# daviyan5/ninpol

Measured on AMD Instinct MI355X. Metric: Mnodes/s interpolated (GLS, 10M-cell hex mesh) + achieved HBM GB/s vs peak, higher is better.
Workload: dtype f64

## Files before the change

include/ninpol_amd.h:

```cpp
#ifndef NINPOL_AMD_H
#define NINPOL_AMD_H

#include <stdint.h>

#ifdef __cplusplus
extern "C" {
#endif

typedef struct nin_grid nin_grid;

enum {
    NIN_OK = 0,
    NIN_EINVAL = -1,
    NIN_ENOMEM = -2,
    NIN_EHIP = -3,
    NIN_ENODEVICE = -4,
    NIN_ERANGE = -5,
    NIN_ESTATE = -6
};

enum { NIN_METHOD_GLS = 0, NIN_METHOD_IDW = 1, NIN_METHOD_LS = 2 };

enum { NIN_I64 = 0, NIN_F64 = 1 };

const char *nin_last_error(void);
const char *nin_version(void);

int nin_grid_create(int64_t dim, int64_t n_elems, int64_t n_points,
                    const int64_t *npoel, const int64_t *nfael, const int64_t *lnofa,
                    const int64_t *lpofa, const int64_t *nedel, const int64_t *lpoed,
                    const int64_t *connectivity, const int64_t *element_types,
                    const double *coords, int coords_dim, int build_edges, int num_threads,
                    nin_grid **out);
void nin_grid_destroy(nin_grid *g);

int nin_grid_create_on_device(int64_t dim, int64_t n_elems, int64_t n_points,
                              const int64_t *npoel, const int64_t *nfael, const int64_t *lnofa,
                              const int64_t *lpofa, const int64_t *nedel, const int64_t *lpoed,
                              const int64_t *connectivity, const int64_t *element_types,
                              const double *coords, int coords_dim, int build_edges, int device,
                              nin_grid **out);

int64_t nin_grid_scalar(const nin_grid *g, const char *name);

int nin_grid_array_info(nin_grid *g, const char *name, int64_t *count, int *dtype);
int nin_grid_array_copy(nin_grid *g, const char *name, void *dst, int64_t count);

int nin_device_count(int *count);
int nin_grid_to_device(nin_grid *g, int device);
int nin_grid_device(const nin_grid *g);

int nin_grid_update_points(nin_grid *g, const double *xyz, int coords_dim);
int nin_grid_update_points_device(nin_grid *g, const double *dev_xyz, int coords_dim, void *stream);
int64_t nin_grid_geometry_updates(const nin_grid *g);
int nin_grid_has_transpose_index(const nin_grid *g);

int nin_fields_set(nin_grid *g, const double *permeability, const double *diff_mag,
                   const double *neumann_flag, const double *neumann_val);

int nin_fields_set_permeability_device(nin_grid *g, const double *dev_permeability, const double *dev_scale, void *stream);
int nin_fields_get_permeability(nin_grid *g, double *permeability, double *diff_mag);
int64_t nin_grid_field_updates(const nin_grid *g);

int nin_fields_scatter_permeability_device(nin_grid *g, const void *dev_cell_ids, int ids_are_int64, int64_t n,
                                           const double *dev_permeability, const double *dev_scale, void *stream);
int nin_weights_dirty_device(nin_grid *g, int method, int add_neumann, double *dev_csr_data, double *dev_neumann_ws, void *stream,
                             int clear, int64_t *n_recomputed);
int64_t nin_grid_dirty_nodes(nin_grid *g);
int nin_grid_dirty_reset(nin_grid *g, int all_dirty, void *stream);

int nin_grid_scatter_points_device(nin_grid *g, const void *dev_node_ids, int ids_are_int64, int64_t n, const double *dev_xyz,
                                   int coords_dim, void *stream);
int nin_grid_scatter_points(nin_grid *g, const int64_t *node_ids, int64_t n, const double *xyz, int coords_dim);

int nin_fields_set_flags_device(nin_grid *g, const void *dev_flags, int flags_are_bytes, void *stream);
int nin_fields_scatter_flags_device(nin_grid *g, const void *dev_node_ids, int ids_are_int64, int64_t n,
                                    const void *dev_flags, int flags_are_bytes, void *stream);
int nin_fields_get_flags(nin_grid *g, uint8_t *neumann );
int64_t nin_grid_flag_updates(const nin_grid *g);

int nin_weights_device(nin_grid *g, int method, const int64_t *targets, int64_t n_targets,
                       int add_neumann, double *dev_csr_data, double *dev_neumann_ws, void *stream);

int nin_weights_host(nin_grid *g, int method, const int64_t *targets, int64_t n_targets,
                     int add_neumann, double *csr_data, double *neumann_ws);

int nin_csr_compact_host(nin_grid *g, const double *dev_csr_data, int32_t *indptr, int32_t *indices,
                         double *data, int64_t *nnz_out, void *stream);

int nin_interpolate_csr_host(nin_grid *g, int method, int32_t *indptr, int32_t *indices, double *data,
                             int64_t *nnz_out, double *neumann_ws);

typedef struct nin_hostmatrix nin_hostmatrix;
int nin_hostmatrix_create(nin_grid *g, int method, nin_hostmatrix **out);
int nin_hostmatrix_full(nin_hostmatrix *m, int32_t *indptr, int32_t *indices, double *data, double *neumann_ws, int64_t *nnz_out,
                        void *stream);
int nin_hostmatrix_update(nin_hostmatrix *m, int clear, void *stream, int64_t *n_rows, int64_t *n_changed, int64_t *n_entries);
int nin_hostmatrix_patch(nin_hostmatrix *m, const int32_t *indptr, int32_t *indices, double *data, double *neumann_ws,
                         int32_t *out_indptr, int32_t *out_indices, double *out_data);
void nin_hostmatrix_destroy(nin_hostmatrix *m);

int nin_csr_patch_rows(int64_t P, const int32_t *indptr, int32_t *indices, double *data, double *neumann_ws, int64_t m,
                       const int32_t *nodes, const int32_t *counts, const int32_t *off, const int32_t *pack_indices,
                       const double *pack_data, const double *pack_nws, int32_t *out_indptr, int32_t *out_indices, double *out_data);

int nin_apply_host(nin_grid *g, int method, const double *u_cells, double *node_values, double *neumann_ws);

int nin_apply_device(nin_grid *g, int method, const double *dev_u_cells, int32_t n_fields, double *dev_node_values,
                     double *dev_neumann_ws, void *stream);
int nin_apply_fields_host(nin_grid *g, int method, const double *u_cells, int32_t n_fields, double *node_values,
                          double *neumann_ws);

int nin_spmv_device(nin_grid *g, const double *dev_csr_data, const double *dev_u_cells, int32_t n_fields, double *dev_node_values,
                    void *stream);
int nin_spmv_transpose_device(nin_grid *g, const double *dev_csr_data, const double *dev_node_values, int32_t n_fields,
                              double *dev_cell_values, void *stream);
int nin_apply_transpose_fields_host(nin_grid *g, int method, const double *node_values, int32_t n_fields, double *cell_values);

int nin_gls_weights_backward_device(nin_grid *g, int add_neumann, const double *dev_grad_csr, const double *dev_grad_neumann_ws,
                                    double *dev_grad_perm, double *dev_grad_diff_mag, void *stream);
int nin_sddmm_device(nin_grid *g, const double *dev_u_cells, const double *dev_node_values, int32_t n_fields, double *dev_grad_csr,
                     void *stream);
int nin_gls_permeability_gradient_host(nin_grid *g, const double *node_values, const double *cell_values, int32_t n_fields,
                                       double *grad_permeability);
int nin_gls_adjoint_plan(nin_grid *g, int64_t counts[4]);
int nin_gls_weights_tangent_device(nin_grid *g, int add_neumann, int32_t n_tangents, const double *dev_tangent_perm,
                                   const double *dev_tangent_diff_mag, double *dev_tangent_csr, double *dev_tangent_neumann_ws,
                                   void *stream);
int nin_gls_permeability_tangent_host(nin_grid *g, const double *tangent_permeability, const double *cell_values, int32_t n_fields,
                                      double *node_values, double *neumann_ws);

int nin_gls_weights_backward_points_device(nin_grid *g, int add_neumann, const double *dev_grad_csr, const double *dev_grad_neumann_ws,
                                           double *dev_grad_points, void *stream);
int nin_gls_points_gradient_host(nin_grid *g, const double *node_values, const double *cell_values, int32_t n_fields,
                                 double *grad_points);

int nin_gls_weights_tangent_points_device(nin_grid *g, int add_neumann, int32_t n_tangents, const double *dev_tangent_points,
                                          double *dev_tangent_csr, double *dev_tangent_neumann_ws, void *stream);
int nin_gls_points_tangent_host(nin_grid *g, const double *tangent_points, const double *cell_values, int32_t n_fields,
                                double *node_values, double *neumann_ws);

typedef struct nin_gls_jacobian nin_gls_jacobian;
int nin_gls_jacobian_create(nin_grid *g, nin_gls_jacobian **out);
int nin_gls_jacobian_linearize(nin_gls_jacobian *J, const double *dev_u_cells, const double *dev_neumann_values, void *stream);
int nin_gls_jacobian_apply(nin_gls_jacobian *J, int32_t n, const double *dev_dperm, const double *dev_ddiff_mag, double *dev_dnode,
                           void *stream);
int nin_gls_jacobian_apply_transpose(nin_gls_jacobian *J, int32_t n, const double *dev_v, double *dev_grad_perm,
                                     double *dev_grad_diff_mag, void *stream);
int nin_gls_jacobian_contrib(nin_gls_jacobian *J, const double **dev_contrib, const double **dev_fold);
int nin_gls_jacobian_stamp(const nin_gls_jacobian *J, int64_t stamp[3]);
void nin_gls_jacobian_destroy(nin_gls_jacobian *J);
int nin_gls_jacobian_linearize_host(nin_gls_jacobian *J, const double *u_cells, const double *neumann_values);
int nin_gls_jacobian_apply_host(nin_gls_jacobian *J, int32_t n, const double *dperm, const double *ddiff_mag, double *dnode);
int nin_gls_jacobian_apply_transpose_host(nin_gls_jacobian *J, int32_t n, const double *v, double *grad_perm, double *grad_diff_mag);
int nin_gls_jacobian_fetch_host(nin_gls_jacobian *J, double *contrib, double *fold);

typedef struct nin_gls_rjacobian nin_gls_rjacobian;
int nin_gls_rjacobian_create(nin_grid *g, int32_t n_params, nin_gls_rjacobian **out);
int nin_gls_rjacobian_linearize(nin_gls_rjacobian *J, const double *dev_u_cells, const double *dev_neumann_values, const double *dev_basis,
                                int32_t basis_per_cell, void *stream);
int nin_gls_rjacobian_apply(nin_gls_rjacobian *J, int32_t n, const double *dev_dtheta, double *dev_dnode, void *stream);
int nin_gls_rjacobian_apply_transpose(nin_gls_rjacobian *J, int32_t n, const double *dev_v, double *dev_grad_theta, void *stream);
int nin_gls_rjacobian_buffer(nin_gls_rjacobian *J, const double **dev_R, int32_t *n_params);
int nin_gls_rjacobian_stamp(const nin_gls_rjacobian *J, int64_t stamp[3]);
void nin_gls_rjacobian_destroy(nin_gls_rjacobian *J);
int nin_gls_rjacobian_linearize_host(nin_gls_rjacobian *J, const double *u_cells, const double *neumann_values, const double *basis,
                                     int32_t basis_per_cell);
int nin_gls_rjacobian_apply_host(nin_gls_rjacobian *J, int32_t n, const double *dtheta, double *dnode);
int nin_gls_rjacobian_apply_transpose_host(nin_gls_rjacobian *J, int32_t n, const double *v, double *grad_theta);
int nin_gls_rjacobian_fetch_host(nin_gls_rjacobian *J, double *R);

typedef struct nin_gls_xjacobian nin_gls_xjacobian;
int nin_gls_xjacobian_create(nin_grid *g, nin_gls_xjacobian **out);
int nin_gls_xjacobian_linearize(nin_gls_xjacobian *J, const double *dev_u_cells, const double *dev_neumann_values, void *stream);
int nin_gls_xjacobian_apply(nin_gls_xjacobian *J, int32_t n, const double *dev_dpoints, double *dev_dnode, void *stream);
int nin_gls_xjacobian_apply_transpose(nin_gls_xjacobian *J, int32_t n, const double *dev_v, double *dev_grad_points, void *stream);
int nin_gls_xjacobian_records(nin_gls_xjacobian *J, const double **dev_cell, const double **dev_face, const double **dev_own,
                              int64_t *scratch_bytes);
int nin_gls_xjacobian_stamp(const nin_gls_xjacobian *J, int64_t stamp[3]);
void nin_gls_xjacobian_destroy(nin_gls_xjacobian *J);
int nin_gls_xjacobian_linearize_host(nin_gls_xjacobian *J, const double *u_cells, const double *neumann_values);
int nin_gls_xjacobian_apply_host(nin_gls_xjacobian *J, int32_t n, const double *dpoints, double *dnode);
int nin_gls_xjacobian_apply_transpose_host(nin_gls_xjacobian *J, int32_t n, const double *v, double *grad_points);
int nin_gls_xjacobian_fetch_host(nin_gls_xjacobian *J, double *cell, double *face, double *own);

int nin_gls_xjacobian_pattern(nin_gls_xjacobian *J, int64_t *n_blocks, const int64_t **dev_block_ptr, const int32_t **dev_block_col,
                              void *stream);
int nin_gls_xjacobian_pattern_copy(nin_gls_xjacobian *J, int64_t *dev_block_ptr_out, int32_t *dev_block_col_out, void *stream);
int nin_gls_xjacobian_assemble(nin_gls_xjacobian *J, double *dev_values, void *stream);
int nin_gls_xjacobian_pattern_host(nin_gls_xjacobian *J, int64_t *block_ptr, int32_t *block_col, int64_t *n_blocks);
int nin_gls_xjacobian_assemble_host(nin_gls_xjacobian *J, double *values);

int nin_gls_jacobian_linearize_dirty(nin_gls_jacobian *J, const double *dev_u_cells, const double *dev_neumann_values, void *stream, int clear,
                                     int64_t *n_rows);
int nin_gls_rjacobian_linearize_dirty(nin_gls_rjacobian *J, const double *dev_u_cells, const double *dev_neumann_values, const double *dev_basis,
                                      int32_t basis_per_cell, void *stream, int clear, int64_t *n_rows);
int nin_gls_xjacobian_linearize_dirty(nin_gls_xjacobian *J, const double *dev_u_cells, const double *dev_neumann_values, void *stream, int clear,
                                      int64_t *n_rows);
int nin_gls_jacobian_linearize_dirty_host(nin_gls_jacobian *J, const double *u_cells, const double *neumann_values, int clear, int64_t *n_rows);
int nin_gls_rjacobian_linearize_dirty_host(nin_gls_rjacobian *J, const double *u_cells, const double *neumann_values, const double *basis,
                                           int32_t basis_per_cell, int clear, int64_t *n_rows);
int nin_gls_xjacobian_linearize_dirty_host(nin_gls_xjacobian *J, const double *u_cells, const double *neumann_values, int clear, int64_t *n_rows);
int nin_grid_mark_dirty_device(nin_grid *g, const void *dev_ids, int ids_are_int64, int64_t n, int ids_are_cells, void *stream);

int nin_pack_connectivity(int32_t n_blocks, const int64_t *const *block_data, const int64_t *rows, const int64_t *cols,
                          const int64_t *type_id, int64_t *connectivity, int64_t *element_types);
int nin_pack_table_row(const double *src, int64_t n, int64_t src_cols, int64_t take, double *dst);
int nin_diff_mag(const double *permeability, int64_t n_elems, double *diff_mag);
int nin_hash64(const void *data, size_t bytes, uint64_t *out);

int nin_host_alloc(size_t bytes, void **ptr);
int nin_host_free(void *ptr);

int nin_grid_release_scratch(nin_grid *g);

int64_t nin_algorithmic_bytes(const nin_grid *g, int method);

const char *nin_kernel_name(int method);

int nin_gls_plan(const nin_grid *g, int64_t counts[22]);

int nin_gls_plan_flops(nin_grid *g, double alg[22], double ref[22], int64_t computed[22]);

#define NIN_EXCHANGE_HANDLE_BYTES 64
typedef struct nin_exchange nin_exchange;
int nin_exchange_create(int device, int rank, int world, size_t slot_bytes, nin_exchange **out);
void nin_exchange_destroy(nin_exchange *x);
int nin_exchange_handle(nin_exchange *x, void *handle64);
int nin_exchange_connect(nin_exchange *x, const void *all_handles);
int nin_exchange_push(nin_exchange *x, const void *dev_src, size_t bytes, size_t offset, void *stream);
int nin_exchange_wait_sent(nin_exchange *x, void *stream, int host_wait);
void *nin_exchange_buffer(nin_exchange *x);
size_t nin_exchange_slot_bytes(const nin_exchange *x);

#ifdef __cplusplus
}
#endif
#endif
```

ninpol_amd/_lib.py:

```python
import ctypes
import os

HERE = os.path.dirname(os.path.abspath(__file__))
LIB_PATH = os.environ.get("NINPOL_AMD_LIB") or os.path.join(HERE, "libninpol_amd.so")

NIN_OK = 0
NIN_EINVAL, NIN_ENOMEM, NIN_EHIP, NIN_ENODEVICE, NIN_ERANGE, NIN_ESTATE = -1, -2, -3, -4, -5, -6
METHOD_ID = {"gls": 0, "idw": 1, "ls": 2}

EXPORTS = (
    "nin_last_error", "nin_version", "nin_grid_create", "nin_grid_create_on_device", "nin_grid_destroy", "nin_grid_scalar",
    "nin_grid_array_info", "nin_grid_array_copy", "nin_device_count", "nin_grid_to_device", "nin_grid_device",
    "nin_fields_set", "nin_weights_device", "nin_weights_host", "nin_csr_compact_host", "nin_interpolate_csr_host", "nin_apply_host",
    "nin_apply_device", "nin_apply_fields_host", "nin_spmv_device", "nin_spmv_transpose_device", "nin_apply_transpose_fields_host",
    "nin_pack_connectivity", "nin_pack_table_row", "nin_diff_mag",
    "nin_algorithmic_bytes", "nin_kernel_name", "nin_gls_plan", "nin_gls_plan_flops", "nin_host_alloc", "nin_host_free", "nin_hash64",
    "nin_grid_release_scratch",
    "nin_grid_update_points", "nin_grid_update_points_device", "nin_grid_geometry_updates", "nin_grid_has_transpose_index",
    "nin_fields_set_permeability_device", "nin_fields_get_permeability", "nin_grid_field_updates",
    "nin_fields_scatter_permeability_device", "nin_weights_dirty_device", "nin_grid_dirty_nodes", "nin_grid_dirty_reset",
    "nin_grid_scatter_points_device", "nin_grid_scatter_points",
    "nin_fields_set_flags_device", "nin_fields_scatter_flags_device", "nin_fields_get_flags", "nin_grid_flag_updates",
    "nin_hostmatrix_create", "nin_hostmatrix_full", "nin_hostmatrix_update", "nin_hostmatrix_patch", "nin_hostmatrix_destroy",
    "nin_csr_patch_rows",
    "nin_gls_weights_backward_device", "nin_sddmm_device", "nin_gls_adjoint_plan", "nin_gls_permeability_gradient_host",
    "nin_gls_weights_tangent_device", "nin_gls_permeability_tangent_host",
    "nin_gls_weights_backward_points_device", "nin_gls_points_gradient_host",
    "nin_gls_weights_tangent_points_device", "nin_gls_points_tangent_host",
    "nin_gls_jacobian_create", "nin_gls_jacobian_linearize", "nin_gls_jacobian_apply", "nin_gls_jacobian_apply_transpose",
    "nin_gls_jacobian_contrib", "nin_gls_jacobian_stamp", "nin_gls_jacobian_destroy", "nin_gls_jacobian_linearize_host",
    "nin_gls_jacobian_apply_host", "nin_gls_jacobian_apply_transpose_host", "nin_gls_jacobian_fetch_host",
    "nin_gls_rjacobian_create", "nin_gls_rjacobian_linearize", "nin_gls_rjacobian_apply", "nin_gls_rjacobian_apply_transpose",
    "nin_gls_rjacobian_buffer", "nin_gls_rjacobian_stamp", "nin_gls_rjacobian_destroy", "nin_gls_rjacobian_linearize_host",
    "nin_gls_rjacobian_apply_host", "nin_gls_rjacobian_apply_transpose_host", "nin_gls_rjacobian_fetch_host",
    "nin_gls_xjacobian_create", "nin_gls_xjacobian_linearize", "nin_gls_xjacobian_apply", "nin_gls_xjacobian_apply_transpose",
    "nin_gls_xjacobian_records", "nin_gls_xjacobian_stamp", "nin_gls_xjacobian_destroy", "nin_gls_xjacobian_linearize_host",
    "nin_gls_xjacobian_apply_host", "nin_gls_xjacobian_apply_transpose_host", "nin_gls_xjacobian_fetch_host",
    "nin_gls_xjacobian_pattern", "nin_gls_xjacobian_pattern_copy", "nin_gls_xjacobian_assemble", "nin_gls_xjacobian_pattern_host",
    "nin_gls_xjacobian_assemble_host",
    "nin_gls_jacobian_linearize_dirty", "nin_gls_rjacobian_linearize_dirty", "nin_gls_xjacobian_linearize_dirty",
    "nin_gls_jacobian_linearize_dirty_host", "nin_gls_rjacobian_linearize_dirty_host", "nin_gls_xjacobian_linearize_dirty_host",
    "nin_grid_mark_dirty_device",
    "nin_exchange_create", "nin_exchange_destroy", "nin_exchange_handle", "nin_exchange_connect", "nin_exchange_push",
    "nin_exchange_wait_sent", "nin_exchange_buffer", "nin_exchange_slot_bytes",
)

_lib = None


class NinpolError(RuntimeError):
    def __init__(self, code, text):
        super().__init__(f"libninpol_amd error {code}: {text}")
        self.code = code
        self.text = text


def load():
    global _lib
    if _lib is not None:
        return _lib
    if not os.path.exists(LIB_PATH):
        raise ImportError(f"{LIB_PATH} is missing: build it with `python -m ninpol_amd.build` "
                          "(there is no CPU fallback for the weight kernels)")
    L = ctypes.CDLL(LIB_PATH)
    vp, i64, i32, cp, dp = ctypes.c_void_p, ctypes.c_int64, ctypes.c_int, ctypes.c_char_p, ctypes.c_void_p
    L.nin_last_error.restype = cp
    L.nin_version.restype = cp
    L.nin_grid_create.argtypes = [i64, i64, i64] + [vp] * 9 + [i32, i32, i32, ctypes.POINTER(vp)]
    L.nin_grid_create_on_device.argtypes = [i64, i64, i64] + [vp] * 9 + [i32, i32, i32, ctypes.POINTER(vp)]
    L.nin_grid_destroy.argtypes = [vp]
    L.nin_grid_destroy.restype = None
    L.nin_grid_scalar.argtypes = [vp, cp]
    L.nin_grid_scalar.restype = i64
    L.nin_grid_array_info.argtypes = [vp, cp, ctypes.POINTER(i64), ctypes.POINTER(i32)]
    L.nin_grid_array_copy.argtypes = [vp, cp, vp, i64]
    L.nin_device_count.argtypes = [ctypes.POINTER(i32)]
    L.nin_grid_to_device.argtypes = [vp, i32]
    L.nin_grid_device.argtypes = [vp]
    L.nin_fields_set.argtypes = [vp, dp, dp, dp, dp]
    L.nin_weights_device.argtypes = [vp, i32, vp, i64, i32, vp, vp, vp]
    L.nin_weights_host.argtypes = [vp, i32, vp, i64, i32, vp, vp]
    L.nin_csr_compact_host.argtypes = [vp, vp, vp, vp, vp, ctypes.POINTER(i64), vp]
    L.nin_interpolate_csr_host.argtypes = [vp, i32, vp, vp, vp, ctypes.POINTER(i64), vp]
    L.nin_apply_host.argtypes = [vp, i32, vp, vp, vp]
    L.nin_apply_device.argtypes = [vp, i32, vp, i32, vp, vp, vp]
    L.nin_apply_fields_host.argtypes = [vp, i32, vp, i32, vp, vp]
    L.nin_spmv_device.argtypes = [vp, vp, vp, i32, vp, vp]
    L.nin_spmv_transpose_device.argtypes = [vp, vp, vp, i32, vp, vp]
    L.nin_apply_transpose_fields_host.argtypes = [vp, i32, vp, i32, vp]
    L.nin_gls_weights_backward_device.argtypes = [vp, i32, vp, vp, vp, vp, vp]
    L.nin_sddmm_device.argtypes = [vp, vp, vp, i32, vp, vp]
    L.nin_gls_adjoint_plan.argtypes = [vp, vp]
    L.nin_gls_permeability_gradient_host.argtypes = [vp, vp, vp, i32, vp]
    L.nin_gls_weights_tangent_device.argtypes = [vp, i32, i32, vp, vp, vp, vp, vp]
    L.nin_gls_permeability_tangent_host.argtypes = [vp, vp, vp, i32, vp, vp]
    L.nin_gls_weights_backward_points_device.argtypes = [vp, i32, vp, vp, vp, vp]
    L.nin_gls_points_gradient_host.argtypes = [vp, vp, vp, i32, vp]
    L.nin_gls_weights_tangent_points_device.argtypes = [vp, i32, i32, vp, vp, vp, vp]
    L.nin_gls_points_tangent_host.argtypes = [vp, vp, vp, i32, vp, vp]
    L.nin_gls_jacobian_create.argtypes = [vp, ctypes.POINTER(vp)]
    L.nin_gls_jacobian_linearize.argtypes = [vp, vp, vp, vp]
    L.nin_gls_jacobian_apply.argtypes = [vp, i32, vp, vp, vp, vp]
    L.nin_gls_jacobian_apply_transpose.argtypes = [vp, i32, vp, vp, vp, vp]
    L.nin_gls_jacobian_contrib.argtypes = [vp, ctypes.POINTER(vp), ctypes.POINTER(vp)]
    L.nin_gls_jacobian_stamp.argtypes = [vp, vp]
    L.nin_gls_jacobian_destroy.argtypes = [vp]
    L.nin_gls_jacobian_destroy.restype = None
    L.nin_gls_jacobian_linearize_host.argtypes = [vp, vp, vp]
    L.nin_gls_jacobian_apply_host.argtypes = [vp, i32, vp, vp, vp]
    L.nin_gls_jacobian_apply_transpose_host.argtypes = [vp, i32, vp, vp, vp]
    L.nin_gls_jacobian_fetch_host.argtypes = [vp, vp, vp]
    L.nin_gls_rjacobian_create.argtypes = [vp, i32, ctypes.POINTER(vp)]
    L.nin_gls_rjacobian_linearize.argtypes = [vp, vp, vp, vp, i32, vp]
    L.nin_gls_rjacobian_apply.argtypes = [vp, i32, vp, vp, vp]
    L.nin_gls_rjacobian_apply_transpose.argtypes = [vp, i32, vp, vp, vp]
    L.nin_gls_rjacobian_buffer.argtypes = [vp, ctypes.POINTER(vp), ctypes.POINTER(i32)]
    L.nin_gls_rjacobian_stamp.argtypes = [vp, vp]
    L.nin_gls_rjacobian_destroy.argtypes = [vp]
    L.nin_gls_rjacobian_destroy.restype = None
    L.nin_gls_rjacobian_linearize_host.argtypes = [vp, vp, vp, vp, i32]
    L.nin_gls_rjacobian_apply_host.argtypes = [vp, i32, vp, vp]
    L.nin_gls_rjacobian_apply_transpose_host.argtypes = [vp, i32, vp, vp]
    L.nin_gls_rjacobian_fetch_host.argtypes = [vp, vp]
    L.nin_gls_xjacobian_create.argtypes = [vp, ctypes.POINTER(vp)]
    L.nin_gls_xjacobian_linearize.argtypes = [vp, vp, vp, vp]
    L.nin_gls_xjacobian_apply.argtypes = [vp, i32, vp, vp, vp]
    L.nin_gls_xjacobian_apply_transpose.argtypes = [vp, i32, vp, vp, vp]
    L.nin_gls_xjacobian_records.argtypes = [vp, ctypes.POINTER(vp), ctypes.POINTER(vp), ctypes.POINTER(vp), ctypes.POINTER(i64)]
    L.nin_gls_xjacobian_stamp.argtypes = [vp, vp]
    L.nin_gls_xjacobian_destroy.argtypes = [vp]
    L.nin_gls_xjacobian_destroy.restype = None
    L.nin_gls_xjacobian_linearize_host.argtypes = [vp, vp, vp]
    L.nin_gls_xjacobian_apply_host.argtypes = [vp, i32, vp, vp]
    L.nin_gls_xjacobian_apply_transpose_host.argtypes = [vp, i32, vp, vp]
    L.nin_gls_xjacobian_fetch_host.argtypes = [vp, vp, vp, vp]
    L.nin_gls_xjacobian_pattern.argtypes = [vp, ctypes.POINTER(i64), ctypes.POINTER(vp), ctypes.POINTER(vp), vp]
    L.nin_gls_xjacobian_pattern_copy.argtypes = [vp, vp, vp, vp]
    L.nin_gls_xjacobian_assemble.argtypes = [vp, vp, vp]
    L.nin_gls_xjacobian_pattern_host.argtypes = [vp, vp, vp, ctypes.POINTER(i64)]
    L.nin_gls_xjacobian_assemble_host.argtypes = [vp, vp]
    L.nin_gls_jacobian_linearize_dirty.argtypes = [vp, vp, vp, vp, i32, ctypes.POINTER(i64)]
    L.nin_gls_rjacobian_linearize_dirty.argtypes = [vp, vp, vp, vp, i32, vp, i32, ctypes.POINTER(i64)]
    L.nin_gls_xjacobian_linearize_dirty.argtypes = [vp, vp, vp, vp, i32, ctypes.POINTER(i64)]
    L.nin_gls_jacobian_linearize_dirty_host.argtypes = [vp, vp, vp, i32, ctypes.POINTER(i64)]
    L.nin_gls_rjacobian_linearize_dirty_host.argtypes = [vp, vp, vp, vp, i32, i32, ctypes.POINTER(i64)]
    L.nin_gls_xjacobian_linearize_dirty_host.argtypes = [vp, vp, vp, i32, ctypes.POINTER(i64)]
    L.nin_grid_mark_dirty_device.argtypes = [vp, vp, i32, i64, i32, vp]
    L.nin_pack_connectivity.argtypes = [i32, vp, vp, vp, vp, vp, vp]
    L.nin_pack_table_row.argtypes = [vp, i64, i64, i64, vp]
    L.nin_diff_mag.argtypes = [vp, i64, vp]
    L.nin_algorithmic_bytes.argtypes = [vp, i32]
    L.nin_algorithmic_bytes.restype = i64
    L.nin_kernel_name.argtypes = [i32]
    L.nin_kernel_name.restype = cp
    L.nin_gls_plan.argtypes = [vp, vp]
    L.nin_gls_plan_flops.argtypes = [vp, vp, vp, vp]
    L.nin_host_alloc.argtypes = [ctypes.c_size_t, ctypes.POINTER(vp)]
    L.nin_host_free.argtypes = [vp]
    L.nin_hash64.argtypes = [vp, ctypes.c_size_t, ctypes.POINTER(ctypes.c_uint64)]
    L.nin_grid_release_scratch.argtypes = [vp]
    L.nin_grid_update_points.argtypes = [vp, vp, i32]
    L.nin_grid_update_points_device.argtypes = [vp, vp, i32, vp]
    L.nin_grid_geometry_updates.argtypes = [vp]
    L.nin_grid_geometry_updates.restype = i64
    L.nin_grid_has_transpose_index.argtypes = [vp]
    L.nin_fields_set_permeability_device.argtypes = [vp, vp, vp, vp]
    L.nin_fields_get_permeability.argtypes = [vp, vp, vp]
    L.nin_grid_field_updates.argtypes = [vp]
    L.nin_grid_field_updates.restype = i64
    L.nin_fields_scatter_permeability_device.argtypes = [vp, vp, i32, i64, vp, vp, vp]
    L.nin_grid_scatter_points_device.argtypes = [vp, vp, i32, i64, vp, i32, vp]
    L.nin_grid_scatter_points.argtypes = [vp, vp, i64, vp, i32]
    L.nin_fields_set_flags_device.argtypes = [vp, vp, i32, vp]
    L.nin_fields_scatter_flags_device.argtypes = [vp, vp, i32, i64, vp, i32, vp]
    L.nin_fields_get_flags.argtypes = [vp, vp]
    L.nin_grid_flag_updates.argtypes = [vp]
    L.nin_grid_flag_updates.restype = i64
    L.nin_weights_dirty_device.argtypes = [vp, i32, i32, vp, vp, vp, i32, ctypes.POINTER(i64)]
    L.nin_grid_dirty_nodes.argtypes = [vp]
    L.nin_grid_dirty_nodes.restype = i64
    L.nin_grid_dirty_reset.argtypes = [vp, i32, vp]
    L.nin_hostmatrix_create.argtypes = [vp, i32, ctypes.POINTER(vp)]
    L.nin_hostmatrix_full.argtypes = [vp, vp, vp, vp, vp, ctypes.POINTER(i64), vp]
    L.nin_hostmatrix_update.argtypes = [vp, i32, vp, ctypes.POINTER(i64), ctypes.POINTER(i64), ctypes.POINTER(i64)]
    L.nin_hostmatrix_patch.argtypes = [vp] * 8
    L.nin_hostmatrix_destroy.argtypes = [vp]
    L.nin_hostmatrix_destroy.restype = None
    L.nin_csr_patch_rows.argtypes = [i64, vp, vp, vp, vp, i64] + [vp] * 9
    L.nin_exchange_create.argtypes = [i32, i32, i32, ctypes.c_size_t, ctypes.POINTER(vp)]
    L.nin_exchange_destroy.argtypes = [vp]
    L.nin_exchange_destroy.restype = None
    L.nin_exchange_handle.argtypes = [vp, vp]
    L.nin_exchange_connect.argtypes = [vp, vp]
    L.nin_exchange_push.argtypes = [vp, vp, ctypes.c_size_t, ctypes.c_size_t, vp]
    L.nin_exchange_wait_sent.argtypes = [vp, vp, i32]
    L.nin_exchange_buffer.argtypes = [vp]
    L.nin_exchange_buffer.restype = vp
    L.nin_exchange_slot_bytes.argtypes = [vp]
    L.nin_exchange_slot_bytes.restype = ctypes.c_size_t
    _lib = L
    return L


def check(rc):
    if rc != NIN_OK:
        raise NinpolError(rc, load().nin_last_error().decode())


def _ptr(a):
    return None if a is None else a.ctypes.data_as(ctypes.c_void_p)


def _vp(address):
    return ctypes.c_void_p(address) if address else None


def device_count():
    n = ctypes.c_int(0)
    rc = load().nin_device_count(ctypes.byref(n))
    return n.value if rc == NIN_OK else 0


class PinnedPool:

    def __init__(self, keep_bytes=None):
        self.free = []
        if keep_bytes is None:
            keep_bytes = int(os.environ.get("NINPOL_AMD_PINNED_KEEP_BYTES", 4 << 30))
        self.keep_bytes = int(keep_bytes)

    def idle_bytes(self):
        return sum(b for b, _ in self.free)

    def trim(self, to_bytes=0):
        self.free.sort()
        while self.free and self.idle_bytes() > to_bytes:
            _, addr = self.free.pop()
            load().nin_host_free(addr)

    def empty(self, n, dtype):
        import weakref
        import numpy as np
        nbytes = max(int(n) * np.dtype(dtype).itemsize, 1)
        best = None
        for i, (b, _) in enumerate(self.free):
            if nbytes <= b <= 2 * nbytes + 4096 and (best is None or b < self.free[best][0]):
                best = i
        if best is not None:
            size, addr = self.free.pop(best)
        else:
            p = ctypes.c_void_p()
            if load().nin_host_alloc(nbytes, ctypes.byref(p)) != 0 or not p.value:
                return np.empty(int(n), dtype=dtype)
            size, addr = nbytes, p.value
        owner = (ctypes.c_char * size).from_address(addr)
        weakref.finalize(owner, self._release, size, addr)
        return np.frombuffer(owner, dtype=dtype, count=int(n))

    def _release(self, size, addr):
        try:
            if sum(b for b, _ in self.free) + size <= self.keep_bytes:
                self.free.append((size, addr))
            else:
                load().nin_host_free(addr)
        except Exception:
            pass
```

ninpol_amd/build.py:

```python
import os
import shutil
import subprocess
import sys

HERE = os.path.dirname(os.path.abspath(__file__))
CSRC = os.path.join(HERE, "csrc")
OBJ = os.path.join(CSRC, "_obj")
LIB = os.path.join(HERE, "libninpol_amd.so")
ROCM = os.environ.get("ROCM_PATH", "/opt/rocm")
ARCH = "gfx950"

UNITS = [
    ("grid_host.cpp", "g++", ["-fopenmp", "-ffp-contract=off"]),
    ("pack_host.cpp", "g++", ["-fopenmp", "-ffp-contract=off"]),
    ("kernels_idw_ls.hip", "hipcc", ["-ffp-contract=off"]),
    ("kernels_gls.hip", "hipcc", []),
    ("kernels_gls_block.hip", "hipcc", []),
    ("kernels_gls_hex8mf.hip", "hipcc", ["-mllvm", "-amdgpu-atomic-optimizer-strategy=None"]),
    ("kernels_gls_mfw.hip", "hipcc", []),
    ("kernels_gls_mfx.hip", "hipcc", []),
    ("kernels_gls_mfg.hip", "hipcc", []),
    ("kernels_gls_quad4.hip", "hipcc", []),
    ("kernels_gls_adjoint.hip", "hipcc", []),
    ("kernels_gls_shape.hip", "hipcc", []),
    ("kernels_gls_jacobian.hip", "hipcc", []),
    ("kernels_gls_jacobian_reduced.hip", "hipcc", []),
    ("kernels_gls_shape_jacobian.hip", "hipcc", []),
    ("kernels_gls_shape_assemble.hip", "hipcc", []),
    ("kernels_csr.hip", "hipcc", []),
    ("csr_dirty.hip", "hipcc", []),
    ("csr_patch.cpp", "g++", ["-fopenmp"]),
    ("grid_device.hip", "hipcc", ["-ffp-contract=off"]),
    ("grid_update.hip", "hipcc", ["-ffp-contract=off"]),
    ("grid_scatter.hip", "hipcc", ["-ffp-contract=off"]),
    ("fields_update.hip", "hipcc", ["-ffp-contract=off"]),
    ("fields_scatter.hip", "hipcc", ["-ffp-contract=off"]),
    ("flags_update.hip", "hipcc", []),
    ("jacobian_dirty.hip", "hipcc", []),
    ("abi_grid.hip", "hipcc", ["-Wno-unknown-pragmas"]),
    ("abi_plan.hip", "hipcc", ["-Wno-unknown-pragmas"]),
    ("abi_update.hip", "hipcc", ["-Wno-unknown-pragmas"]),
    ("abi_csr.hip", "hipcc", ["-Wno-unknown-pragmas"]),
    ("abi_apply.hip", "hipcc", ["-Wno-unknown-pragmas"]),
    ("abi_jacobian.hip", "hipcc", ["-Wno-unknown-pragmas"]),
    ("abi_jacobian_reduced.hip", "hipcc", ["-Wno-unknown-pragmas"]),
    ("abi_jacobian_points.hip", "hipcc", ["-Wno-unknown-pragmas"]),
    ("abi_jacobian_dirty.hip", "hipcc", ["-Wno-unknown-pragmas"]),
    ("exchange.hip", "hipcc", []),
]


def _run(cmd):
    print("+", " ".join(cmd), flush=True)
    subprocess.check_call(cmd)


def _hipcc():
    return shutil.which("hipcc") or os.path.join(ROCM, "bin", "hipcc")


def needs_build():
    if not os.path.exists(LIB):
        return True
    t = os.path.getmtime(LIB)
    srcs = [os.path.join(CSRC, f) for f in os.listdir(CSRC) if f.endswith((".hip", ".cpp", ".hpp"))]
    srcs += [os.path.join(os.path.dirname(HERE), "include", "ninpol_amd.h"), os.path.abspath(__file__)]
    return any(os.path.getmtime(s) > t for s in srcs)


def build(force=False, verbose_resources=False):
    if not force and not needs_build():
        return LIB
    os.makedirs(OBJ, exist_ok=True)
    objs = []
    for src, cc, extra in UNITS:
        obj = os.path.join(OBJ, os.path.splitext(src)[0] + ".o")
        common = ["-O3", "-fPIC", "-std=c++17", "-c", os.path.join(CSRC, src), "-o", obj]
        if cc == "hipcc":
            cmd = [_hipcc(), f"--offload-arch={ARCH}"] + extra + os.environ.get("NIN_EXTRA_HIPCC_FLAGS", "").split() + common
            if verbose_resources:
                cmd.insert(1, "-Rpass-analysis=kernel-resource-usage")
        else:
            cmd = [cc, "-I", os.path.join(ROCM, "include")] + extra + common
        _run(cmd)
        objs.append(obj)
    _run(["g++", "-shared", "-o", LIB] + objs +
         ["-L", os.path.join(ROCM, "lib"), "-lamdhip64", "-lgomp", "-Wl,-rpath," + os.path.join(ROCM, "lib")])
    build_tools()
    return LIB


def build_tools():
    tools = os.path.join(os.path.dirname(HERE), "tools")
    os.makedirs(os.path.join(tools, "_bin"), exist_ok=True)
    for name in ("test_xstrip", "test_face_tau"):
        _run([_hipcc(), f"--offload-arch={ARCH}", "-O3", "-std=c++17", "-I", CSRC, os.path.join(tools, name + ".hip"), "-o",
              os.path.join(tools, "_bin", name)])


if __name__ == "__main__":
    print(build(force="--force" in sys.argv, verbose_resources="--resources" in sys.argv))
```

ninpol_amd/csrc/abi_plan.hip:

```cpp
#include <hipcub/hipcub.hpp>
#include <cmath>

#include "abi_internal.hpp"
#include "hex8_desc.hpp"
#include "mfw_desc.hpp"
#include "mfg_desc.hpp"
#include "mfx_desc.hpp"
#include "quad4_desc.hpp"

using namespace nin;

namespace {

#ifndef NIN_LOCALITY_RUN
#define NIN_LOCALITY_RUN 16
#endif
constexpr int kLocalityRun = NIN_LOCALITY_RUN;
__device__ __forceinline__ uint32_t spread10(uint32_t v) {
    v = (v | (v << 16)) & 0x030000FFu;
    v = (v | (v << 8)) & 0x0300F00Fu;
    v = (v | (v << 4)) & 0x030C30C3u;
    v = (v | (v << 2)) & 0x09249249u;
    return v;
}
__global__ void k_locality_keys(const double *__restrict__ coords, const int32_t *__restrict__ nodes, int32_t count, double lo,
                                double scale, int32_t c1, int32_t c2, int32_t c3, int32_t strip, double lscale,
                                uint32_t *__restrict__ keys) {
    const int64_t i = (int64_t)blockIdx.x * blockDim.x + threadIdx.x;
    if (i >= count) return;
    const int32_t p = nodes[i & ~(int64_t)(kLocalityRun - 1)];
    uint32_t q[3];
#pragma unroll
    for (int k = 0; k < 3; ++k) {
        const double t = (coords[3 * (size_t)p + k] - lo) * scale;
        q[k] = t > 0.0 ? (t < 1023.0 ? (uint32_t)t : 1023u) : 0u;
    }
    const int32_t self = nodes[i];
    const uint32_t piece = (uint32_t)(self >= c1) + (uint32_t)(self >= c2) + (uint32_t)(self >= c3);
    if (strip > 0) {
        const double ty = (coords[3 * (size_t)p + 1] - lo) * lscale, tz = (coords[3 * (size_t)p + 2] - lo) * lscale;
        const uint32_t yq = ty > 0.0 ? (ty < 32767.0 ? (uint32_t)(ty + 0.5) : 32767u) : 0u;
        const uint32_t zq = tz > 0.0 ? (tz < 32767.0 ? (uint32_t)(tz + 0.5) : 32767u) : 0u;
        keys[i] = (piece << 30) | ((yq / (uint32_t)strip) << 15) | zq;
        return;
    }
    keys[i] = (piece << 30) | spread10(q[0]) | (spread10(q[1]) << 1) | (spread10(q[2]) << 2);
}
int locality_order(const DeviceGrid &d, int32_t *list, int32_t count, const int32_t *chunk_node) {
    if (count < 2048) return NIN_OK;
    double lo = 0.0, hi = 0.0;
    {
        DevTmp<double> mm;
        DevTmp<void> rt;
        size_t rb = 0, rb2 = 0;
        const int n3 = 3 * d.v.n_points;
        bool ok = hipMalloc((void **)&mm, 16) == hipSuccess &&
                  hipcub::DeviceReduce::Min(nullptr, rb, d.v.coords, mm.p, n3) == hipSuccess &&
                  hipcub::DeviceReduce::Max(nullptr, rb2, d.v.coords, mm.p + 1, n3) == hipSuccess &&
                  hipMalloc(&rt, rb > rb2 ? rb : rb2) == hipSuccess;
        rb = rb > rb2 ? rb : rb2;
        ok = ok && hipcub::DeviceReduce::Min(rt, rb, d.v.coords, mm.p, n3) == hipSuccess &&
             hipcub::DeviceReduce::Max(rt, rb, d.v.coords, mm.p + 1, n3) == hipSuccess;
        double h2[2] = {0.0, 0.0};
        ok = ok && hipMemcpy(h2, mm, 16, hipMemcpyDeviceToHost) == hipSuccess;
        if (!ok) return fail(NIN_EHIP, "locality order: bounding cube: %s", hipGetErrorString(hipGetLastError()));
        lo = h2[0]; hi = h2[1];
    }
    if (!(hi > lo)) return NIN_OK;
    DevTmp<uint32_t> keys, keys_out;
    DevTmp<int32_t> list_out;
    DevTmp<void> tmp;
    size_t tmp_bytes = 0;
    int rc = NIN_OK;
    auto step = [&](hipError_t e) { if (e != hipSuccess && rc == NIN_OK) rc = fail(NIN_EHIP, "locality order: %s", hipGetErrorString(e)); return e == hipSuccess; };
    if (step(hipMalloc((void **)&keys, (size_t)count * 4)) && step(hipMalloc((void **)&keys_out, (size_t)count * 4)) &&
        step(hipMalloc((void **)&list_out, (size_t)count * 4))) {
        const char *mode = getenv("NIN_GLS_LOCALITY_ORDER");
        const int32_t strip = !mode ? 16 : mode[0] == 's' ? (mode[1] ? atoi(mode + 1) : 16) : 0;
        const double levels = std::cbrt((double)d.v.n_points) - 1.0;
        hipLaunchKernelGGL(k_locality_keys, dim3((unsigned)((count + 255) / 256)), dim3(256), 0, nullptr, d.v.coords, list, count, lo,
                           1024.0 / (hi - lo), chunk_node[1], chunk_node[2], chunk_node[3], strip, (levels > 1.0 ? levels : 1.0) / (hi - lo), keys.p);
        if (step(hipGetLastError()) && step(hipcub::DeviceRadixSort::SortPairs(nullptr, tmp_bytes, keys.p, keys_out.p, list, list_out.p, count)) &&
            step(hipMalloc(&tmp, tmp_bytes)) &&
            step(hipcub::DeviceRadixSort::SortPairs(tmp, tmp_bytes, keys.p, keys_out.p, list, list_out.p, count)))
            (void)step(hipMemcpy(list, list_out, (size_t)count * 4, hipMemcpyDeviceToDevice));
    }
    return rc;
}

static_assert(kGlsDescHex8 == kHex8DescWords && kGlsDescQuad4 == kQuad4DescWords && kGlsDescMfw == kMfwDescWords &&
                  kGlsDescMfx == kMfxDescWords && kGlsDescMfg == kMfgDescWords, "gls_plan.hpp's descriptor sizes are not the descriptor headers'");

int launch_plan_desc(const DeviceGrid &d, GlsKernel k, const int32_t *nodes, int32_t count, uint32_t *desc, hipStream_t stream) {
    if (count <= 0) return 0;
    switch (gls_plan_row(k).family) {
        case GlsFamily::hex8: return launch_hex8_desc(d.v, nodes, count, reinterpret_cast<int32_t *>(desc), stream);
        case GlsFamily::quad4: return launch_quad4_desc(d.v, nodes, count, reinterpret_cast<int32_t *>(desc), stream);
        case GlsFamily::mfw: return launch_mfw_desc(d.v, nodes, count, desc, stream);
        case GlsFamily::mfx: return launch_mfx_desc(d.v, nodes, count, desc, stream);
        case GlsFamily::mfg: return launch_mfg_desc(d.v, nodes, count, desc, stream);
        default: return 0;
    }
}

int launch_plan_kernel(const DeviceGrid &d, GlsKernel k, const int32_t *nodes, const uint32_t *desc, int32_t count, int add_neumann,
                       double *out, double *nws, hipStream_t stream) {
    const GlsPlanRow r = gls_plan_row(k);
    const DeviceGrid::GlsList &l = d.plan[k];
    int32_t *queue = r.counter >= 0 ? d.gls_queue + r.counter : nullptr;
    const int32_t *idesc = reinterpret_cast<const int32_t *>(desc);
    switch (r.family) {
        case GlsFamily::block: return launch_gls_block(d.v, nodes, count, l.waves, l.col_slots, l.lds_bytes, add_neumann, out, nws, queue, stream);
        case GlsFamily::scratch:
            return launch_gls_class(d.v, nodes, count, 0, l.rows_per_lane, add_neumann, out, nws, d.gls_scratch, d.gls_scratch_stride,
                                    d.gls_scratch_slots, stream);
        case GlsFamily::hex8: return launch_gls_hex8mf(d.v, nodes, idesc, count, add_neumann, out, nws, queue, stream);
        case GlsFamily::mfw: return launch_gls_mfw(d.v, nodes, desc, count, r.sub, add_neumann, out, nws, queue, stream);
        case GlsFamily::small: return launch_gls_small(d.v, nodes, count, r.sub, add_neumann, out, nws, stream);
        case GlsFamily::quad4: return launch_gls_quad4(d.v, nodes, idesc, count, add_neumann, out, nws, stream);
        case GlsFamily::mfx: return launch_gls_mfx(d.v, nodes, desc, count, r.sub, add_neumann, out, nws, queue, stream);
        case GlsFamily::mfg: return launch_gls_mfg(d.v, nodes, desc, count, add_neumann, out, nws, queue, d.mfg_tiles, d.mfg_slots, stream);
    }
    return NIN_EINVAL;
}

}

int nin::build_gls_plan(nin_grid *g) {
    DeviceGrid &d = g->d;
    const int64_t P = g->h.n_points;
    int rc;
    g->node_class.assign((size_t)P, 0);
    auto unless = [](const char *name, int bit) { return getenv(name) == nullptr ? bit : 0; };
    const int use_group = unless("NIN_GLS_NO_GROUP", kRouteHex8) | unless("NIN_GLS_NO_MFW", kRouteMfw) |
                          unless("NIN_GLS_NO_MFW_GENERAL", kRouteMfwGeneral) | unless("NIN_GLS_NO_SMALL", kRouteSmall) |
                          unless("NIN_GLS_NO_QUAD4", kRouteQuad4) | unless("NIN_GLS_NO_MFX", kRouteMfx) |
                          unless("NIN_GLS_NO_MFX_7X12", kRouteMfx7x12) | unless("NIN_GLS_NO_MFX_SMALL", kRouteMfxSmall) |
                          unless("NIN_GLS_NO_MFG", kRouteMfg) | (getenv("NIN_GLS_MFX_NO_BOUNDARY") != nullptr ? kRouteMfxNoBoundary : 0) |
                          unless("NIN_GLS_MFW_GENERAL", kRouteMfxTakesGeneral);
    const bool force_global = getenv("NIN_GLS_FORCE_GLOBAL") != nullptr;
    int64_t need_max[kGlsClasses] = {0}, rows_max[kGlsClasses] = {0}, cols_max[kGlsClasses] = {0};
    {
        uint8_t *dcls = nullptr;
        DevTmp<unsigned long long> dmax;
        unsigned long long hmax[3 * kGlsClasses];
        if ((rc = dev_alloc(d, &dcls, (size_t)P))) return rc;
        d.node_class = dcls;
        if (hipMalloc((void **)&dmax, sizeof hmax) != hipSuccess) return fail(NIN_ENOMEM, "hipMalloc");
        hipError_t e1 = hipMemset(dmax, 0, sizeof hmax);
        const int lrc = launch_classify(d.v, use_group, force_global, dcls, dmax, nullptr);
        if (e1 == hipSuccess) e1 = hipMemcpy(g->node_class.data(), dcls, (size_t)P, hipMemcpyDeviceToHost);
        if (e1 == hipSuccess) e1 = hipMemcpy(hmax, dmax, sizeof hmax, hipMemcpyDeviceToHost);
        if (lrc || e1 != hipSuccess) return fail(NIN_EHIP, "node classification: %s", hipGetErrorString(e1));
        for (int c = 0; c < kGlsClasses; ++c) { need_max[c] = (int64_t)hmax[3 * c]; rows_max[c] = (int64_t)hmax[3 * c + 1]; cols_max[c] = (int64_t)hmax[3 * c + 2]; }
    }
    std::vector<int32_t> lists[kGlsPlanKernels];
    {
        int8_t kernel_of[256];
        for (int c = 0; c < 256; ++c) kernel_of[c] = (int8_t)gls_class_kernel(c);
        for (int64_t p = 0; p < P; ++p) {
            const int k = kernel_of[g->node_class[p]];
            if (k < 0) return fail(NIN_EHIP, "node classification: class byte %d belongs to no kernel", (int)g->node_class[p]);
            lists[k].push_back((int32_t)p);
        }
        std::vector<int32_t> rest;
        rest.reserve((size_t)P - lists[gk::hex8].size());
        for (int64_t p = 0; p < P; ++p)
            if (g->node_class[p] != gls_class_byte(gk::hex8)) rest.push_back((int32_t)p);
        d.noncube_count = (int32_t)rest.size();
        const int32_t *lp = nullptr;
        if (d.noncube_count && (rc = dev_upload(d, &lp, rest))) return rc;
        d.noncube_nodes = lp;
        d.noncube_nodes_ready = true;
    }
    for (int c = 0; c < kGlsClasses; ++c) {
        auto &k = d.plan[c];
        k.lds_bytes = c == kGlsClasses - 1 ? 0 : (int32_t)need_max[c];
        k.rows_per_lane = (int32_t)std::max<int64_t>(1, (rows_max[c] + 63) / 64);
        k.waves = gls_class_waves(c);
        k.col_slots = (int32_t)std::max<int64_t>(1, (cols_max[c] + 63) / 64);
    }
    constexpr int K = DeviceGrid::kE2eChunks;
    for (int j = 0; j <= K; ++j) d.chunk_node[j] = j == K ? (int32_t)P : (int32_t)((P * j / K) & ~(int64_t)63);
    const char *lo_env = getenv("NIN_GLS_LOCALITY_ORDER");
    const bool locality = !(lo_env && (lo_env[0] == 'o' || lo_env[0] == '0'));
    for (int k = 0; k < kGlsPlanKernels; ++k) {
        auto &l = d.plan[k];
        l.count = (int32_t)lists[k].size();
        for (int j = 0; j <= K; ++j) l.chunk_off[j] = (int32_t)(std::lower_bound(lists[k].begin(), lists[k].end(), d.chunk_node[j]) - lists[k].begin());
        if (!l.count) continue;
        const int32_t *lp = nullptr;
        if ((rc = dev_upload(d, &lp, lists[k]))) return rc;
        l.nodes = const_cast<int32_t *>(lp);
        if (k == gk::hex8 && locality && (rc = locality_order(d, l.nodes, l.count, d.chunk_node))) return rc;
        if (const int words = gls_plan_row(k).desc_words) {
            if ((rc = dev_alloc(d, &l.desc, (size_t)l.count * words))) return rc;
            if (launch_plan_desc(d, GlsKernel(k), l.nodes, l.count, l.desc, nullptr)) return fail(NIN_EHIP, "descriptor kernel of plan kernel %d", k);
        }
    }
    if (d.plan[gk::mfg_tiles].count) {
        d.mfg_slots = std::min<int32_t>(d.plan[gk::mfg_tiles].count, kMfgResidentWaves);
        if ((rc = dev_alloc(d, &d.mfg_tiles, (size_t)d.mfg_slots * kMfgSlotDoubles))) return rc;
    }
    d.gls_too_large = rows_max[gk::scratch] > 1024;
    if ((rc = dev_alloc(d, &d.gls_queue, (size_t)kGlsQueueInts))) return rc;
    if (d.plan[gk::scratch].count) {
        d.gls_scratch_slots = std::min<int32_t>(d.plan[gk::scratch].count, 512);
        d.gls_scratch_stride = need_max[gk::scratch] / 8;
        if ((rc = dev_alloc(d, &d.gls_scratch, (size_t)d.gls_scratch_slots * d.gls_scratch_stride))) return rc;
    }
    const char *mn = getenv("NIN_E2E_MIN_NODES");
    d.chunkable = P >= (mn ? atoll(mn) : 64 * 1024) && P >= 64 * K && getenv("NIN_E2E_NO_PIPELINE") == nullptr;
    for (int c = 0; c < kGlsClasses; ++c)
        if (d.plan[c].count == P) { d.plan[c].nodes = nullptr; d.chunkable = false; }
    return NIN_OK;
}

static constexpr GlsKernel kSideOrder[] = {gk::mfg_tiles, gk::scratch};
static constexpr GlsKernel kMainOrder[] = {gk::hex8,     gk::mfw_large, gk::mfw_small, gk::mfw_general, gk::small4,       gk::small8,
                                           gk::small12,  gk::quad4,     gk::mfx_6x10,  gk::mfx_7x11,    gk::mfx_8x13,     gk::mfx_9x15,
                                           gk::mfx_10x16, gk::mfx_boundary, gk::mfx_4x7, gk::mfx_7x12,  gk::mfg_tiles,    gk::block1,
                                           gk::block2,   gk::block4,    gk::block8,    gk::scratch};
static constexpr bool main_order_is_complete() {
    unsigned seen = 0;
    for (GlsKernel k : kMainOrder) seen |= 1u << k;
    return sizeof kMainOrder / sizeof kMainOrder[0] == kGlsPlanKernels && seen == (1u << kGlsPlanKernels) - 1;
}
static_assert(main_order_is_complete(), "kMainOrder must name every kernel of the plan once");
static bool on_side_stream(GlsKernel k) { return std::find(std::begin(kSideOrder), std::end(kSideOrder), k) != std::end(kSideOrder); }

struct PlanRange { const int32_t *nodes; const uint32_t *desc; int32_t count; };
static PlanRange plan_range(const DeviceGrid &d, GlsKernel k, int piece) {
    const auto &l = d.plan[k];
    const int32_t b = piece < 0 ? 0 : l.chunk_off[piece], n = (piece < 0 ? l.count : l.chunk_off[piece + 1]) - b;
    return {l.nodes ? l.nodes + b : nullptr, l.desc ? l.desc + (size_t)gls_plan_row(k).desc_words * b : nullptr, n};
}

int nin::gls_side_begin(DeviceGrid &d, int piece, int add_neumann, double *out, double *nws, hipStream_t stream) {
    d.side_pending = false;
    bool any = false;
    for (GlsKernel k : kSideOrder) any = any || plan_range(d, k, piece).count > 0;
    if (!any || getenv("NIN_GLS_NO_SIDE_STREAM") != nullptr) return 0;
    if (lazy_stream(d.side_stream) || lazy_event(d.ev_fork) || lazy_event(d.ev_join)) return -3;
    hipStream_t side = static_cast<hipStream_t>(d.side_stream);
    if (hipEventRecord(static_cast<hipEvent_t>(d.ev_fork), stream) != hipSuccess || hipStreamWaitEvent(side, static_cast<hipEvent_t>(d.ev_fork), 0) != hipSuccess)
        return -3;
    int rc = 0;
    for (GlsKernel k : kSideOrder) {
        const PlanRange r = plan_range(d, k, piece);
        if (!rc && r.count > 0) rc = launch_plan_kernel(d, k, r.nodes, r.desc, r.count, add_neumann, out, nws, side);
    }
    if (!rc && hipEventRecord(static_cast<hipEvent_t>(d.ev_join), side) != hipSuccess) rc = -3;
    d.side_pending = rc == 0;
    return rc;
}
static int gls_side_end(DeviceGrid &d, hipStream_t stream) {
    if (!d.side_pending) return 0;
    d.side_pending = false;
    return hipStreamWaitEvent(stream, static_cast<hipEvent_t>(d.ev_join), 0) == hipSuccess ? 0 : -3;
}

int nin::gls_only() {
    const char *e = getenv("NIN_GLS_ONLY");
    return e && *e ? atoi(e) : -1;
}

int nin::gls_main(DeviceGrid &d, int piece, bool cube, int only, int add_neumann, double *out, double *nws, hipStream_t stream) {
    int rc = 0;
    for (GlsKernel k : kMainOrder) {
        if ((k == gk::hex8 && !cube) || (only >= 0 && only != k) || (d.side_pending && on_side_stream(k))) continue;
        const PlanRange r = plan_range(d, k, piece);
        if (!rc && r.count > 0) rc = launch_plan_kernel(d, k, r.nodes, r.desc, r.count, add_neumann, out, nws, stream);
    }
    if (!rc) rc = gls_side_end(d, stream);
    return rc;
}

int nin::launch_lists(DeviceGrid &d, int method, const int32_t *lists, const int32_t *off, uint32_t *desc, const size_t *desc_first,
                      int add_neumann, double *out, double *nws, hipStream_t stream, DirtyLaps *laps) {
    const bool gls = method == NIN_METHOD_GLS;
    if (laps) laps->mark(1);
    if (gls) {
        for (int k = 0; k < kGlsPlanKernels; ++k)
            if (launch_plan_desc(d, GlsKernel(k), lists + off[k], off[k + 1] - off[k], desc + desc_first[k], stream))
                return fail(NIN_EHIP, "descriptor kernel of plan kernel %d", k);
        HIP_TRY(hipMemsetAsync(d.gls_queue, 0, kGlsQueueInts * sizeof(int32_t), stream));
    }
    if (laps) laps->mark(2);
    int rc = 0;
    if (!gls)
        rc = method == NIN_METHOD_IDW ? launch_idw(d.v, lists, off[kGlsPlanKernels], 0, 0, out, nws, stream)
                                      : launch_ls(d.v, lists, off[kGlsPlanKernels], 0, 0, out, nws, stream);
    else
        for (GlsKernel k : kMainOrder)
            if (!rc && off[k + 1] > off[k])
                rc = launch_plan_kernel(d, k, lists + off[k], desc + desc_first[k], off[k + 1] - off[k], add_neumann, out, nws, stream);
    if (rc) return fail(rc, "kernel launch failed: %s", hipGetErrorString(hipGetLastError()));
    if (laps) laps->mark(3);
    return NIN_OK;
}

int nin_weights_device(nin_grid *g, int method, const int64_t *targets, int64_t n_targets, int add_neumann,
                       double *dev_csr_data, double *dev_neumann_ws, void *stream_) {
    if (!g || !dev_csr_data || !dev_neumann_ws) return fail(NIN_EINVAL, "NULL argument");
    DeviceGrid &d = g->d;
    int rc = on_device(g, kHintWeights);
    if (!rc) rc = weights_ready(d, method);
    if (rc) return rc;
    hipStream_t stream = static_cast<hipStream_t>(stream_);
    HIP_TRY(hipSetDevice(d.device));
    const int64_t P = g->h.n_points;
    const bool all = targets == nullptr;
    if (!all && n_targets < 0) return fail(NIN_EINVAL, "negative n_targets");
    if (all) {
        if (method == NIN_METHOD_IDW) rc = launch_idw(d.v, nullptr, (int32_t)P, (int32_t)g->h.mx_elems_per_point, d.nnz_e, dev_csr_data, dev_neumann_ws, stream);
        else if (method == NIN_METHOD_LS) rc = launch_ls(d.v, nullptr, (int32_t)P, (int32_t)g->h.mx_elems_per_point, d.nnz_e, dev_csr_data, dev_neumann_ws, stream);
        else {
            HIP_TRY(hipMemsetAsync(d.gls_queue, 0, kGlsQueueInts * sizeof(int32_t), stream));
            const int only = gls_only();
            if (only < 0) rc = gls_side_begin(d, -1, add_neumann, dev_csr_data, dev_neumann_ws, stream);
            if (!rc) rc = gls_main(d, -1, true, only, add_neumann, dev_csr_data, dev_neumann_ws, stream);
        }
        if (rc) return fail(rc, "kernel launch failed: %s", hipGetErrorString(hipGetLastError()));
        return NIN_OK;
    }
    for (int64_t i = 0; i < n_targets; ++i)
        if (targets[i] < 0 || targets[i] >= P) return fail(NIN_EINVAL, "target %lld out of range", (long long)targets[i]);
    HIP_TRY(hipMemsetAsync(dev_csr_data, 0, (size_t)d.nnz_e * 8, stream));
    HIP_TRY(hipMemsetAsync(dev_neumann_ws, 0, (size_t)P * 8, stream));
    if (n_targets == 0) return NIN_OK;
    const bool gls = method == NIN_METHOD_GLS;
    std::vector<int32_t> lists[kGlsPlanKernels];
    for (int64_t i = 0; i < n_targets; ++i) lists[gls ? gls_class_kernel(g->node_class[targets[i]]) : 0].push_back((int32_t)targets[i]);
    std::vector<int32_t> flat;
    int32_t off[kGlsPlanKernels + 1];
    size_t desc_first[kGlsPlanKernels], words = 0;
    for (int k = 0; k < kGlsPlanKernels; ++k) {
        off[k] = (int32_t)flat.size();
        desc_first[k] = words = desc_align(words);
        flat.insert(flat.end(), lists[k].begin(), lists[k].end());
        if (gls) words += lists[k].size() * (size_t)gls_plan_row(k).desc_words;
    }
    off[kGlsPlanKernels] = (int32_t)flat.size();
    const size_t list_words = desc_align(flat.size());
    DevTmp<int32_t> dl0;
    HIP_TRY(hipMalloc((void **)&dl0, (list_words + words) * 4));
    const hipError_t e = hipMemcpy(dl0, flat.data(), flat.size() * 4, hipMemcpyHostToDevice);
    if (e != hipSuccess) return fail(NIN_EHIP, "hipMemcpy: %s", hipGetErrorString(e));
    rc = launch_lists(d, method, dl0, off, reinterpret_cast<uint32_t *>(dl0 + list_words), desc_first, add_neumann, dev_csr_data,
                      dev_neumann_ws, stream, nullptr);
    const hipError_t sy = hipStreamSynchronize(stream);
    if (sy != hipSuccess) return fail(NIN_EHIP, "target kernels: %s", hipGetErrorString(sy));
    return rc;
}

int nin_weights_host(nin_grid *g, int method, const int64_t *targets, int64_t n_targets, int add_neumann,
                     double *csr_data, double *neumann_ws) {
    if (!g || !csr_data || !neumann_ws) return fail(NIN_EINVAL, "NULL argument");
    DeviceGrid &d = g->d;
    if (int rc = on_device(g, kHintWeights, false)) return rc;
    HIP_TRY(hipSetDevice(d.device));
    const size_t nb = (size_t)std::max<int64_t>(d.nnz_e, 1) * 8, pb = (size_t)g->h.n_points * 8;
    DevTmp<double> dd, dn;
    HIP_TRY(hipMalloc((void **)&dd, nb));
    hipError_t e = hipMalloc((void **)&dn, pb);
    if (e != hipSuccess) return fail(NIN_ENOMEM, "hipMalloc: %s", hipGetErrorString(e));
    int rc = nin_weights_device(g, method, targets, n_targets, add_neumann, dd, dn, nullptr);
    if (!rc) {
        e = hipDeviceSynchronize();
        if (e == hipSuccess) e = hipMemcpy(csr_data, dd, (size_t)d.nnz_e * 8, hipMemcpyDeviceToHost);
        if (e == hipSuccess) e = hipMemcpy(neumann_ws, dn, pb, hipMemcpyDeviceToHost);
        if (e != hipSuccess) rc = fail(NIN_EHIP, "weights kernel / copy back: %s", hipGetErrorString(e));
    }
    return rc;
}

namespace {
double hh_flops(int64_t m, int64_t n_pivot, int64_t n_cols) {
    double f = 0;
    for (int64_t k = 0; k < n_pivot; ++k) {
        const double rows = (double)(m - k);
        f += 2 * rows + 8 + 4 * rows * (double)(n_cols - k - 1);
    }
    return f;
}
double multifrontal_flops(int64_t F, int64_t D, int64_t faces, int64_t free_faces, int64_t neumann_rows = 0) {
    const double face = 52.0 * faces + 15.0 * neumann_rows;
    const double p1 = F * (hh_flops(10, 3, 3 + 9 + 1) + 9 + 54 + 6);
    const int64_t m2 = 7 * F + D + 3 * free_faces + neumann_rows, n2 = 3 * D;
    const double p2 = hh_flops(m2, n2, n2 + 1);
    const double tail = (double)n2 * n2 + F * (2 * 9 + 2) + D * (2 * 3 + 1) + 2 * (m2 - n2) + (F + D) + 1;
    return face + p1 + p2 + tail;
}
double dense_flops(int64_t ne, int64_t n_if, int64_t n_nb) {
    const int64_t m = ne + 3 * n_if + n_nb, n = 3 * ne;
    return 52.0 * n_if + 15.0 * n_nb + hh_flops(m, n, n + 1) + (double)n * n + 7.0 * ne + 2.0 * (m - n) + ne + 1;
}
double dgels_flops(double m, double n, double nrhs) { return 2 * m * n * n - 2 * n * n * n / 3 + nrhs * (4 * m * n - 2 * n * n) + nrhs * n * n; }
}

int nin_gls_plan_flops(nin_grid *g, double alg[22], double ref[22], int64_t computed[22]) {
    if (!g || !alg || !ref || !computed) return fail(NIN_EINVAL, "NULL argument");
    DeviceGrid &d = g->d;
    HostGrid &h = g->h;
    if (int rc = on_device(g, kHintToDevice)) return rc;
    if (!d.fields_set || (!d.flag_staging && !d.flags_host_stale))
        return fail(NIN_ESTATE, "nin_fields_set has not been called (the Neumann flags decide which boundary nodes are computed)");
    if (h.ensure(A_ESUP_PTR | A_ESUP | A_FSUP_PTR | A_FSUP | A_ESUF)) return fail(NIN_EHIP, "mirroring the connectivity failed");
    HIP_TRY(hipSetDevice(d.device));
    {
        const int frc = fetch_flag_bytes(g);
        if (frc) return frc;
    }
    for (int k = 0; k < kGlsPlanKernels; ++k) { alg[k] = ref[k] = 0.0; computed[k] = 0; }
    const int64_t P = h.n_points;
    std::vector<uint32_t> fdq((size_t)P, 0u);
    for (int k = 0; k < kGlsPlanKernels; ++k) {
        const GlsPlanRow row = gls_plan_row(k);
        const auto &l = d.plan[k];
        if (row.fdq_word < 0 || l.count <= 0) continue;
        std::vector<int32_t> hn((size_t)l.count);
        std::vector<uint32_t> hd((size_t)l.count * row.desc_words);
        if (hipMemcpy(hn.data(), l.nodes, hn.size() * 4, hipMemcpyDeviceToHost) != hipSuccess ||
            hipMemcpy(hd.data(), l.desc, hd.size() * 4, hipMemcpyDeviceToHost) != hipSuccess)
            return fail(NIN_EHIP, "reading the descriptors back failed");
        for (int32_t i = 0; i < l.count; ++i) fdq[hn[i]] = hd[(size_t)i * row.desc_words + row.fdq_word] & 0xFFFFFFu;
    }
    for (int64_t p = 0; p < P; ++p) {
        const int k = gls_class_kernel(g->node_class[p]);
        const GlsPlanRow row = gls_plan_row(k);
        const int fl = d.flag_staging[p];
        if ((fl & 1) && !(fl & 2)) continue;
        const int64_t eb = h.esup_ptr[p], ne = h.esup_ptr[p + 1] - eb, fb = h.fsup_ptr[p], nf = h.fsup_ptr[p + 1] - fb;
        int64_t n_if = 0;
        for (int64_t q = fb; q < fb + nf; ++q) {
            const int64_t f = h.fsup[q];
            n_if += h.esuf_ptr[f + 1] - h.esuf_ptr[f] > 1;
        }
        const int64_t n_bf = nf - n_if, n_nb = (fl & 2) ? n_bf : 0;
        const int64_t m = ne + 3 * n_if + n_nb;
        if (n_if == 0 || m < 3 * ne) continue;
        ++computed[k];
        ref[k] += dgels_flops((double)(ne + 3 * nf + n_nb), (double)(3 * ne + 1), (double)(ne + (n_nb ? 1 : 0)));
        if (k == gk::hex8) alg[k] += multifrontal_flops(4, 4, 12, 0);
        else if (row.fdq_word >= 0) {
            const uint32_t w = fdq[p];
            alg[k] += multifrontal_flops(w & 255u, (w >> 8) & 255u, n_if, (w >> 16) & 255u, row.family != GlsFamily::mfw ? n_nb : 0);
        } else if (k == gk::quad4) {
            alg[k] += 52.0 * 4 + 15.0 * 4 + 2 * (hh_flops(8, 3, 3 + 6 + 1) + 9 + 36 + 6) + hh_flops(14, 6, 7) + 36 + 2 * 20 + 2 * 7 + 2 * 8 + 5;
        } else if (k >= gk::block2 && k <= gk::block8) {
            const int n_c = (int)std::min<int64_t>(ne, 64);
            uint64_t adj[64] = {0};
            int nfi[64] = {0};
            uint64_t blocked = 0;
            for (int64_t q = fb; q < fb + nf; ++q) {
                const int64_t f = h.fsup[q], e0 = h.esuf_ptr[f];
                const bool internal = h.esuf_ptr[f + 1] - e0 > 1;
                int ia = -1, ib = -1;
                for (int i = 0; i < n_c; ++i) {
                    if (h.esup[eb + i] == h.esuf[e0]) ia = i;
                    if (internal && h.esup[eb + i] == h.esuf[e0 + 1]) ib = i;
                }
                if (internal && ia >= 0 && ib >= 0) { adj[ia] |= 1ull << ib; adj[ib] |= 1ull << ia; ++nfi[ia]; ++nfi[ib]; }
                else if (!internal && ia >= 0 && n_nb) blocked |= 1ull << ia;
            }
            uint64_t chosen = 0;
            double p1 = 0;
            int64_t rows_gone = 0, Fb = 0;
            for (int i = 0; i < n_c; ++i)
                if (nfi[i] >= 1 && nfi[i] <= 4 && !((blocked >> i) & 1ull) && !(adj[i] & chosen)) {
                    chosen |= 1ull << i;
                    p1 += hh_flops(1 + 3 * nfi[i], 3, 3 + 3 * nfi[i] + 1);
                    rows_gone += 3;
                    ++Fb;
                }
            const int64_t m2 = m - rows_gone, n2 = 3 * (ne - Fb);
            alg[k] += 52.0 * n_if + 15.0 * n_nb + p1 + hh_flops(m2, n2, n2 + 1) + (double)(3 * ne) * (3 * ne) + 7.0 * ne + 2.0 * (m - 3 * ne) + ne + 1;
        } else {
            alg[k] += dense_flops(ne, n_if, n_nb);
        }
    }
    return NIN_OK;
}

int nin_gls_plan(const nin_grid *g, int64_t counts[22]) {
    if (!g || !counts) return fail(NIN_EINVAL, "NULL argument");
    if (int rc = on_device(g, kHintToDevice)) return rc;
    for (int k = 0; k < kGlsPlanKernels; ++k) counts[k] = g->d.plan[k].count;
    return NIN_OK;
}
```

ninpol_amd/csrc/abi_update.hip:

```cpp
#include <new>

#include "abi_internal.hpp"

using namespace nin;

namespace {

struct GeometryMirror : LazyArrays {
    const DeviceGrid *d;
    explicit GeometryMirror(const DeviceGrid *dg) : d(dg) {}
    template <class T>
    static int get(std::vector<T> &dst, const T *src, size_t n, std::string *err) {
        if (!src) { *err = "the device copy is gone"; return -3; }
        dst.resize(n);
        if (n && hipMemcpy(dst.data(), src, n * sizeof(T), hipMemcpyDeviceToHost) != hipSuccess) { *err = "hipMemcpy (device to host)"; return -3; }
        return 0;
    }
    int fetch(HostGrid &h, unsigned which, std::string *err) override {
        if (d->device < 0 || hipSetDevice(d->device) != hipSuccess) { *err = "the grid has no device copy"; return -3; }
        const size_t P = (size_t)h.n_points, E = (size_t)h.n_elems, F = (size_t)h.n_faces;
        int rc = 0;
        if (!rc && (which & A_COORDS)) rc = get(h.coords, d->v.coords, P * 3, err);
        if (!rc && (which & A_CENTROIDS)) rc = get(h.centroids, d->v.centroids, E * 3, err);
        if (!rc && (which & A_FCENTERS)) rc = get(h.faces_centers, d->v.face_center, F * 3, err);
        if (!rc && (which & A_NORMALS)) rc = get(h.normal_faces, d->v.face_normal, F * 3, err);
        if (!rc && (which & A_AREAS)) rc = get(h.faces_areas, const_cast<const double *>(d->up_areas), F, err);
        return rc;
    }
};

}

int nin::ensure_update_inputs(nin_grid *g) {
    DeviceGrid &d = g->d;
    HostGrid &h = g->h;
    if (d.up_inpoel) return NIN_OK;
    LazyArrays::GeometryInputs gi;
    if (h.lazy && h.lazy->lend_geometry_inputs(&gi)) {
        for (void *q : {(void *)gi.inpoel, (void *)gi.etype, (void *)gi.inpofa, (void *)gi.areas}) d.allocs.push_back(q);
        d.up_inpoel = gi.inpoel; d.up_etype = gi.etype; d.up_inpofa = gi.inpofa; d.up_areas = gi.areas;
        d.up_areas_valid = true;
        return NIN_OK;
    }
    std::string err;
    if (h.ensure(A_INPOEL | A_ETYPE | A_INPOFA, &err)) return fail(NIN_EHIP, "mirroring the connectivity: %s", err.c_str());
    int rc = dev_alloc(d, &d.up_inpoel, h.inpoel.size());
    if (!rc) rc = dev_alloc(d, &d.up_etype, h.etype.size());
    if (!rc) rc = dev_alloc(d, &d.up_inpofa, h.inpofa.size());
    if (!rc) rc = dev_alloc(d, &d.up_areas, (size_t)h.n_faces);
    auto up = [&](void *dst, const void *src, size_t bytes) {
        if (!rc && bytes && hipMemcpy(dst, src, bytes, hipMemcpyHostToDevice) != hipSuccess) rc = fail(NIN_EHIP, "uploading the connectivity failed");
    };
    up(d.up_inpoel, h.inpoel.data(), h.inpoel.size() * 4);
    up(d.up_etype, h.etype.data(), h.etype.size());
    up(d.up_inpofa, h.inpofa.data(), h.inpofa.size() * 4);
    if (rc) { dev_release(d, d.up_inpoel); dev_release(d, d.up_etype); dev_release(d, d.up_inpofa); dev_release(d, d.up_areas); return rc; }
    d.up_areas_valid = false;
    return NIN_OK;
}

namespace {

uint64_t pack_npoel8(const HostGrid &h) {
    uint64_t npoel8 = 0;
    for (int t = 0; t < kNumElementTypes; ++t) npoel8 |= (uint64_t)(h.npoel[t] & 0xff) << (8 * t);
    return npoel8;
}

int finish_geometry_update(nin_grid *g, int rc, bool on_host, hipStream_t stream, const char *what) {
    DeviceGrid &d = g->d;
    if (!rc && hipEventRecord(static_cast<hipEvent_t>(d.ev_geom), stream) != hipSuccess) rc = fail(NIN_EHIP, "hipEventRecord");
    if (on_host || rc) {
        const hipError_t e = hipStreamSynchronize(stream);
        if (e != hipSuccess && !rc) rc = fail(NIN_EHIP, "%s: %s", what, hipGetErrorString(e));
    }
    g->h.have &= ~A_GEOMETRY;
    if (!g->h.lazy) g->h.lazy.reset(new GeometryMirror(&g->d));
    ++d.geom_updates;
    return rc;
}

int update_points_on_device(nin_grid *g, const double *xyz, bool on_host, int cd, hipStream_t stream) {
    DeviceGrid &d = g->d;
    HostGrid &h = g->h;
    HIP_TRY(hipSetDevice(d.device));
    int rc = ensure_update_inputs(g);
    if (!rc) rc = lazy_event(d.ev_geom);
    if (rc) return rc;
    const size_t P = (size_t)h.n_points;
    double *coords = const_cast<double *>(d.v.coords);
    DevTmp<double> staged;
    if (on_host && cd == 3) {
        HIP_TRY(hipMemcpy(coords, xyz, P * 24, hipMemcpyHostToDevice));
    } else {
        if (on_host) {
            HIP_TRY(hipMalloc((void **)&staged, P * cd * sizeof(double)));
            if (hipMemcpy(staged, xyz, P * cd * sizeof(double), hipMemcpyHostToDevice) != hipSuccess) rc = fail(NIN_EHIP, "uploading the coordinates failed");
        }
        if (!rc && launch_update_coords(on_host ? staged.p : xyz, cd, (int64_t)P, coords, stream)) rc = fail(NIN_EHIP, "coordinate copy: %s", hipGetErrorString(hipGetLastError()));
    }
    const uint64_t npoel8 = pack_npoel8(h);
    if (!rc && launch_update_geometry(d.v, npoel8, d.up_inpoel, d.up_etype, d.up_inpofa, const_cast<double *>(d.v.centroids),
                                      const_cast<double *>(d.v.face_center), const_cast<float *>(d.v.face_normal), d.up_areas, stream))
        rc = fail(NIN_EHIP, "geometry kernels: %s", hipGetErrorString(hipGetLastError()));
    if (!rc && d.v.centroids4 && launch_pad_centroids(d.v.centroids, h.n_elems, const_cast<double *>(d.v.centroids4), stream))
        rc = fail(NIN_EHIP, "centroid padding kernel");
    rc = finish_geometry_update(g, rc, on_host, stream, "geometry update");
    d.up_areas_valid = true;
    d.all_dirty = true;
    return rc;
}

}

int nin_grid_update_points(nin_grid *g, const double *xyz, int coords_dim) {
    if (!g || !xyz) return fail(NIN_EINVAL, "NULL argument");
    if (coords_dim != g->coords_dim) return fail(NIN_EINVAL, "coords_dim %d is not the grid's (%d)", coords_dim, g->coords_dim);
    if (g->d.device >= 0) return update_points_on_device(g, xyz, true, coords_dim, nullptr);
    try {
        g->h.update_points(xyz, coords_dim);
    } catch (const std::bad_alloc &) {
        return fail(NIN_ENOMEM, "out of host memory while updating the geometry");
    }
    return NIN_OK;
}

int nin_grid_update_points_device(nin_grid *g, const double *dev_xyz, int coords_dim, void *stream) {
    if (!g || !dev_xyz) return fail(NIN_EINVAL, "NULL argument");
    if (coords_dim != g->coords_dim) return fail(NIN_EINVAL, "coords_dim %d is not the grid's (%d)", coords_dim, g->coords_dim);
    if (int rc = on_device(g, " (call nin_grid_to_device first, or nin_grid_update_points with a host array)")) return rc;
    return update_points_on_device(g, dev_xyz, false, coords_dim, static_cast<hipStream_t>(stream));
}

int64_t nin_grid_geometry_updates(const nin_grid *g) { return g ? g->d.geom_updates : 0; }

int nin_fields_set_permeability_device(nin_grid *g, const double *dev_permeability, const double *dev_scale, void *stream) {
    if (!g || !dev_permeability) return fail(NIN_EINVAL, "NULL argument");
    if (int rc = on_device(g, " (call nin_grid_to_device first, or nin_fields_set with host arrays)")) return rc;
    DeviceGrid &d = g->d;
    HIP_TRY(hipSetDevice(d.device));
    const hipError_t e = launch_update_permeability(d.v.n_elems, dev_permeability, dev_scale, const_cast<double *>(d.v.perm),
                                                    const_cast<double *>(d.v.diff_mag), static_cast<hipStream_t>(stream));
    if (e != hipSuccess) return fail(NIN_EHIP, "permeability kernel: %s", hipGetErrorString(e));
    d.have_perm = true;
    d.all_dirty = true;
    ++d.field_updates;
    return NIN_OK;
}

int nin_fields_get_permeability(nin_grid *g, double *permeability, double *diff_mag) {
    if (!g) return fail(NIN_EINVAL, "NULL grid");
    if (int rc = on_device(g, kHintToDevice)) return rc;
    DeviceGrid &d = g->d;
    if (!d.have_perm) return fail(NIN_ESTATE, "no permeability is resident (nin_fields_set or nin_fields_set_permeability_device first)");
    HIP_TRY(hipSetDevice(d.device));
    HIP_TRY(hipDeviceSynchronize());
    const size_t E = (size_t)g->h.n_elems;
    if (permeability) HIP_TRY(hipMemcpy(permeability, d.v.perm, E * 9 * 8, hipMemcpyDeviceToHost));
    if (diff_mag) HIP_TRY(hipMemcpy(diff_mag, d.v.diff_mag, E * 8, hipMemcpyDeviceToHost));
    return NIN_OK;
}

int64_t nin_grid_field_updates(const nin_grid *g) { return g ? g->d.field_updates : 0; }

int nin::ensure_dirty_state(DeviceGrid &d, int64_t P) {
    if (d.dirty) return NIN_OK;
    int rc = dev_alloc(d, &d.dirty, (size_t)P);
    if (!rc) rc = dev_alloc(d, &d.dirty_hdr, (size_t)kDirtyHdrInts);
    if (!rc && (hipMemset(d.dirty, 0, (size_t)P) != hipSuccess || hipMemset(d.dirty_hdr, 0, kDirtyHdrInts * sizeof(int32_t)) != hipSuccess))
        rc = fail(NIN_EHIP, "zeroing the dirty set failed");
    if (rc) { dev_release(d, d.dirty); dev_release(d, d.dirty_hdr); }
    return rc;
}

int nin_fields_scatter_permeability_device(nin_grid *g, const void *dev_cell_ids, int ids_are_int64, int64_t n, const double *dev_permeability,
                                           const double *dev_scale, void *stream) {
    if (!g) return fail(NIN_EINVAL, "NULL grid");
    if (n < 0) return fail(NIN_EINVAL, "negative n");
    if (int rc = on_device(g, kHintToDevice)) return rc;
    if (n == 0) return NIN_OK;
    if (!dev_cell_ids || !dev_permeability) return fail(NIN_EINVAL, "NULL argument");
    DeviceGrid &d = g->d;
    if (!d.have_perm) return fail(NIN_ESTATE, "no permeability is resident to patch (nin_fields_set or nin_fields_set_permeability_device first)");
    HIP_TRY(hipSetDevice(d.device));
    int rc = ensure_update_inputs(g);
    if (!rc) rc = ensure_dirty_state(d, g->h.n_points);
    if (rc) return rc;
    rc = launch_scatter_permeability(d.v, pack_npoel8(g->h), d.up_inpoel, d.up_etype, dev_cell_ids, ids_are_int64, n, dev_permeability, dev_scale,
                                     d.dirty, d.dirty_hdr + kDirtyHdrRejected, static_cast<hipStream_t>(stream));
    if (rc) return fail(rc, "scatter kernel: %s", hipGetErrorString(hipGetLastError()));
    d.scattered_cells = true;
    ++d.field_updates;
    return NIN_OK;
}

int nin_fields_set_flags_device(nin_grid *g, const void *dev_flags, int flags_are_bytes, void *stream) {
    if (!g || !dev_flags) return fail(NIN_EINVAL, "NULL argument");
    if (int rc = on_device(g, " (call nin_grid_to_device first, or nin_fields_set with host arrays)")) return rc;
    DeviceGrid &d = g->d;
    HIP_TRY(hipSetDevice(d.device));
    int rc = ensure_dirty_state(d, g->h.n_points);
    if (rc) return rc;
    rc = launch_set_flags(d.v.n_points, dev_flags, flags_are_bytes, const_cast<uint8_t *>(d.v.flags), d.all_dirty ? nullptr : d.dirty,
                          static_cast<hipStream_t>(stream));
    if (rc) return fail(rc, "flag kernel: %s", hipGetErrorString(hipGetLastError()));
    d.fields_set = true;
    d.flags_host_stale = true;
    ++d.flag_updates;
    return NIN_OK;
}

int nin_fields_scatter_flags_device(nin_grid *g, const void *dev_node_ids, int ids_are_int64, int64_t n, const void *dev_flags,
                                    int flags_are_bytes, void *stream) {
    if (!g) return fail(NIN_EINVAL, "NULL grid");
    if (n < 0) return fail(NIN_EINVAL, "negative n");
    if (int rc = on_device(g, kHintToDevice)) return rc;
    if (n == 0) return NIN_OK;
    if (!dev_node_ids || !dev_flags) return fail(NIN_EINVAL, "NULL argument");
    DeviceGrid &d = g->d;
    if (!d.fields_set) return fail(NIN_ESTATE, "no Neumann flags are resident to patch (nin_fields_set or nin_fields_set_flags_device first)");
    HIP_TRY(hipSetDevice(d.device));
    int rc = ensure_dirty_state(d, g->h.n_points);
    if (rc) return rc;
    rc = launch_scatter_flags(d.v.n_points, dev_node_ids, ids_are_int64, n, dev_flags, flags_are_bytes, const_cast<uint8_t *>(d.v.flags),
                              d.all_dirty ? nullptr : d.dirty, d.dirty_hdr + kDirtyHdrRejected, static_cast<hipStream_t>(stream));
    if (rc) return fail(rc, "flag scatter kernel: %s", hipGetErrorString(hipGetLastError()));
    d.scattered_flags = true;
    d.flags_host_stale = true;
    ++d.flag_updates;
    return NIN_OK;
}

int nin::fetch_flag_bytes(nin_grid *g) {
    DeviceGrid &d = g->d;
    if (d.flag_staging && !d.flags_host_stale) return NIN_OK;
    const size_t P = (size_t)g->h.n_points;
    if (!d.flag_staging) HIP_TRY(hipHostMalloc((void **)&d.flag_staging, std::max<size_t>(P, 1), hipHostMallocDefault));
    HIP_TRY(hipDeviceSynchronize());
    HIP_TRY(hipMemcpy(d.flag_staging, d.v.flags, P, hipMemcpyDeviceToHost));
    d.flags_host_stale = false;
    return NIN_OK;
}

int nin_fields_get_flags(nin_grid *g, uint8_t *neumann) {
    if (!g || !neumann) return fail(NIN_EINVAL, "NULL argument");
    if (int rc = on_device(g, kHintToDevice)) return rc;
    DeviceGrid &d = g->d;
    if (!d.fields_set) return fail(NIN_ESTATE, "no Neumann flags are resident (nin_fields_set or nin_fields_set_flags_device first)");
    HIP_TRY(hipSetDevice(d.device));
    d.flags_host_stale = true;
    const int rc = fetch_flag_bytes(g);
    if (rc) return rc;
    const int64_t P = g->h.n_points;
    for (int64_t p = 0; p < P; ++p) neumann[p] = (uint8_t)((d.flag_staging[p] >> 1) & 1);
    return NIN_OK;
}

int64_t nin_grid_flag_updates(const nin_grid *g) { return g ? g->d.flag_updates : 0; }

static int scatter_points_on_device(nin_grid *g, const void *ids, int ids_are_int64, int64_t n, const double *xyz, bool on_host, int cd,
                                    hipStream_t stream) {
    DeviceGrid &d = g->d;
    HostGrid &h = g->h;
    HIP_TRY(hipSetDevice(d.device));
    int rc = ensure_update_inputs(g);
    if (!rc) rc = ensure_dirty_state(d, h.n_points);
    if (rc) return rc;
    if (!d.up_areas_valid) {
        std::string err;
        if (h.ensure(A_AREAS, &err)) return fail(NIN_EHIP, "mirroring faces_areas: %s", err.c_str());
        if (h.n_faces > 0) HIP_TRY(hipMemcpy(d.up_areas, h.faces_areas.data(), (size_t)h.n_faces * sizeof(double), hipMemcpyHostToDevice));
        d.up_areas_valid = true;
    }
    if ((rc = lazy_event(d.ev_geom))) return rc;
    DevTmp<void> staged_ids;
    DevTmp<double> staged_xyz;
    if (on_host) {
        const size_t ib = (size_t)n * sizeof(int64_t), xb = (size_t)n * cd * sizeof(double);
        HIP_TRY(hipMalloc(&staged_ids, ib));
        if (hipMalloc((void **)&staged_xyz, xb) != hipSuccess) rc = fail(NIN_ENOMEM, "hipMalloc(%zu bytes) for the moved rows", xb);
        if (!rc && (hipMemcpy(staged_ids, ids, ib, hipMemcpyHostToDevice) != hipSuccess ||
                    hipMemcpy(staged_xyz, xyz, xb, hipMemcpyHostToDevice) != hipSuccess))
            rc = fail(NIN_EHIP, "uploading the moved nodes failed");
        if (rc) return rc;
        ids = staged_ids; xyz = staged_xyz;
    }
    if (launch_scatter_points(d.v, pack_npoel8(h), d.up_inpoel, d.up_etype, d.up_inpofa, ids, ids_are_int64, n, xyz, cd, d.up_areas, d.dirty,
                              d.dirty_hdr + kDirtyHdrRejected, stream))
        rc = fail(NIN_EHIP, "local geometry kernels: %s", hipGetErrorString(hipGetLastError()));
    d.scattered_nodes = true;
    return finish_geometry_update(g, rc, on_host, stream, "local geometry update");
}

int nin_grid_scatter_points_device(nin_grid *g, const void *dev_node_ids, int ids_are_int64, int64_t n, const double *dev_xyz, int coords_dim,
                                   void *stream) {
    if (!g) return fail(NIN_EINVAL, "NULL grid");
    if (n < 0) return fail(NIN_EINVAL, "negative n");
    if (coords_dim != g->coords_dim) return fail(NIN_EINVAL, "coords_dim %d is not the grid's (%d)", coords_dim, g->coords_dim);
    if (int rc = on_device(g, " (call nin_grid_to_device first, or nin_grid_scatter_points with host arrays)")) return rc;
    if (n == 0) return NIN_OK;
    if (!dev_node_ids || !dev_xyz) return fail(NIN_EINVAL, "NULL argument");
    return scatter_points_on_device(g, dev_node_ids, ids_are_int64, n, dev_xyz, false, coords_dim, static_cast<hipStream_t>(stream));
}

int nin_grid_scatter_points(nin_grid *g, const int64_t *node_ids, int64_t n, const double *xyz, int coords_dim) {
    if (!g) return fail(NIN_EINVAL, "NULL grid");
    if (n < 0) return fail(NIN_EINVAL, "negative n");
    if (coords_dim != g->coords_dim) return fail(NIN_EINVAL, "coords_dim %d is not the grid's (%d)", coords_dim, g->coords_dim);
    if (n == 0) return NIN_OK;
    if (!node_ids || !xyz) return fail(NIN_EINVAL, "NULL argument");
    HostGrid &h = g->h;
    int64_t bad = 0, first = 0;
    for (int64_t i = 0; i < n; ++i)
        if (node_ids[i] < 0 || node_ids[i] >= h.n_points) { if (!bad++) first = node_ids[i]; }
    if (bad) return fail(NIN_EINVAL, "%lld of %lld node ids lie outside [0, %lld) (the first: %lld); nothing was moved", (long long)bad, (long long)n,
                         (long long)h.n_points, (long long)first);
    if (g->d.device >= 0) return scatter_points_on_device(g, node_ids, 1, n, xyz, true, coords_dim, nullptr);
    try {
        for (int64_t i = 0; i < n; ++i)
            for (int k = 0; k < coords_dim && k < 3; ++k) h.coords[(size_t)node_ids[i] * 3 + k] = xyz[i * coords_dim + k];
        const std::vector<double> moved(h.coords);
        h.update_points(moved.data(), 3);
    } catch (const std::bad_alloc &) {
        return fail(NIN_ENOMEM, "out of host memory while updating the geometry");
    }
    return NIN_OK;
}

int nin_grid_mark_dirty_device(nin_grid *g, const void *dev_ids, int ids_are_int64, int64_t n, int ids_are_cells, void *stream) {
    if (!g) return fail(NIN_EINVAL, "NULL grid");
    if (n < 0) return fail(NIN_EINVAL, "negative n");
    if (int rc = on_device(g, kHintToDevice)) return rc;
    if (n == 0) return NIN_OK;
    if (!dev_ids) return fail(NIN_EINVAL, "NULL argument");
    DeviceGrid &d = g->d;
    HIP_TRY(hipSetDevice(d.device));
    int rc = ids_are_cells ? ensure_update_inputs(g) : NIN_OK;
    if (!rc) rc = ensure_dirty_state(d, g->h.n_points);
    if (rc) return rc;
    rc = launch_mark_dirty(d.v, pack_npoel8(g->h), d.up_inpoel, d.up_etype, dev_ids, ids_are_int64, n, ids_are_cells, d.dirty,
                           d.dirty_hdr + kDirtyHdrRejected, static_cast<hipStream_t>(stream));
    if (rc) return fail(rc, "mark kernel: %s", hipGetErrorString(hipGetLastError()));
    d.scattered_marks = true;
    return NIN_OK;
}

int nin::dirty_ids_refused(nin_grid *g, int32_t count, hipStream_t stream) {
    DeviceGrid &d = g->d;
    HIP_TRY(hipMemsetAsync(d.dirty_hdr + kDirtyHdrRejected, 0, sizeof(int32_t), stream));
    const bool nodes = d.scattered_nodes || d.scattered_marks, flags = d.scattered_flags,
               cells = d.scattered_cells || d.scattered_marks || !(nodes || flags);
    d.scattered_cells = d.scattered_nodes = d.scattered_flags = d.scattered_marks = false;
    char who[240];
    if (cells && (nodes || flags))
        snprintf(who, sizeof who, "cell ids outside [0, %lld) or node ids outside [0, %lld) were given to the local updates%s",
                 (long long)g->h.n_elems, (long long)g->h.n_points, flags ? " (nin_fields_scatter_flags_device among them)" : "");
    else if (nodes && flags)
        snprintf(who, sizeof who, "node ids outside [0, %lld) were given to nin_grid_scatter_points_device or nin_fields_scatter_flags_device",
                 (long long)g->h.n_points);
    else if (flags)
        snprintf(who, sizeof who, "node ids outside [0, %lld) were given to nin_fields_scatter_flags_device", (long long)g->h.n_points);
    else if (nodes)
        snprintf(who, sizeof who, "node ids outside [0, %lld) were given to nin_grid_scatter_points_device", (long long)g->h.n_points);
    else
        snprintf(who, sizeof who, "cell ids outside [0, %lld) were given to nin_fields_scatter_permeability_device", (long long)g->h.n_elems);
    return fail(NIN_EINVAL, "%d %s and written nowhere; nothing was launched, the dirty set is kept", (int)count, who);
}

int nin_weights_dirty_device(nin_grid *g, int method, int add_neumann, double *dev_csr_data, double *dev_neumann_ws, void *stream_, int clear,
                             int64_t *n_recomputed) {
    if (n_recomputed) *n_recomputed = 0;
    if (!g || !dev_csr_data || !dev_neumann_ws) return fail(NIN_EINVAL, "NULL argument");
    DeviceGrid &d = g->d;
    int rc = on_device(g, kHintWeights);
    if (!rc) rc = weights_ready(d, method);
    if (rc) return rc;
    const bool gls = method == NIN_METHOD_GLS;
    hipStream_t stream = static_cast<hipStream_t>(stream_);
    HIP_TRY(hipSetDevice(d.device));
    const int32_t P = (int32_t)g->h.n_points;
    int32_t hdr[kDirtyHdrInts] = {0};
    DirtyLaps laps(stream);
    laps.mark(0);
    if (d.dirty) {
        if (!d.all_dirty) {
            const size_t ints = 2 * dirty_compact_hist_ints(P);
            size_t tmp_bytes = 0;
            if (dirty_compact_tmp_bytes(P, &tmp_bytes)) return fail(NIN_EHIP, "sizing the scan of the dirty set failed");
            if (!d.dirty_hist && (rc = dev_alloc(d, &d.dirty_hist, ints))) return rc;
            if (!d.dirty_lists && (rc = dev_alloc(d, &d.dirty_lists, (size_t)P))) return rc;
            if ((rc = grow(d, reinterpret_cast<char **>(&d.dirty_tmp), &d.dirty_tmp_bytes, std::max<size_t>(tmp_bytes, 16)))) return rc;
            if (launch_dirty_compact(P, gls ? 0 : 1, clear, d.dirty, d.node_class, d.dirty_hdr + kDirtyHdrRejected, d.dirty_hist,
                                     d.dirty_hist + ints / 2, d.dirty_tmp, d.dirty_tmp_bytes, d.dirty_lists, d.dirty_hdr, stream))
                return fail(NIN_EHIP, "compacting the dirty set: %s", hipGetErrorString(hipGetLastError()));
        }
        HIP_TRY(hipMemcpyAsync(hdr, d.dirty_hdr, sizeof hdr, hipMemcpyDeviceToHost, stream));
        HIP_TRY(hipStreamSynchronize(stream));
        if (hdr[kDirtyHdrRejected] != 0) return dirty_ids_refused(g, hdr[kDirtyHdrRejected], stream);
        d.scattered_cells = d.scattered_nodes = d.scattered_flags = d.scattered_marks = false;
    }
    if (d.all_dirty) {
        if ((rc = nin_weights_device(g, method, nullptr, 0, add_neumann, dev_csr_data, dev_neumann_ws, stream_))) return rc;
        if (clear) {
            if (d.dirty) HIP_TRY(hipMemsetAsync(d.dirty, 0, (size_t)P, stream));
            d.all_dirty = false;
        }
        if (n_recomputed) *n_recomputed = P;
        return NIN_OK;
    }
    const int32_t *off = hdr + kDirtyHdrOffsets;
    const int32_t total = off[kGlsPlanKernels];
    if (total < 0 || total > P) return fail(NIN_EHIP, "the dirty set's lists hold %d nodes of %d", (int)total, (int)P);
    if (n_recomputed) *n_recomputed = total;
    if (total == 0) return NIN_OK;
    size_t desc_first[kGlsPlanKernels], words = 0;
    for (int k = 0; gls && k < kGlsPlanKernels; ++k) {
        if (off[k + 1] < off[k]) return fail(NIN_EHIP, "the dirty set's lists are out of order");
        desc_first[k] = words = desc_align(words);
        words += (size_t)(off[k + 1] - off[k]) * (size_t)gls_plan_row(k).desc_words;
    }
    if (words > d.dirty_desc_words && (rc = grow(d, &d.dirty_desc, &d.dirty_desc_words, words + words / 2))) return rc;
    if ((rc = launch_lists(d, method, d.dirty_lists, off, d.dirty_desc, desc_first, add_neumann, dev_csr_data, dev_neumann_ws, stream, &laps)))
        return rc;
    laps.report(total);
    return NIN_OK;
}

int64_t nin_grid_dirty_nodes(nin_grid *g) {
    if (!g || g->d.device < 0 || g->d.prebuilt) return 0;
    DeviceGrid &d = g->d;
    if (d.all_dirty) return -1;
    if (!d.dirty) return 0;
    int32_t n = 0;
    if (hipSetDevice(d.device) != hipSuccess || hipDeviceSynchronize() != hipSuccess ||
        hipMemset(d.dirty_hdr + kDirtyHdrCount, 0, sizeof(int32_t)) != hipSuccess ||
        launch_dirty_count((int32_t)g->h.n_points, d.dirty, d.dirty_hdr + kDirtyHdrCount, nullptr) ||
        hipMemcpy(&n, d.dirty_hdr + kDirtyHdrCount, sizeof n, hipMemcpyDeviceToHost) != hipSuccess) {
        (void)fail(NIN_EHIP, "counting the dirty nodes: %s", hipGetErrorString(hipGetLastError()));
        return -2;
    }
    return n;
}

int nin_grid_dirty_reset(nin_grid *g, int all_dirty, void *stream) {
    if (!g) return fail(NIN_EINVAL, "NULL grid");
    DeviceGrid &d = g->d;
    if (int rc = on_device(g, kHintToDevice)) return rc;
    HIP_TRY(hipSetDevice(d.device));
    if (!all_dirty && d.dirty) {
        HIP_TRY(hipMemsetAsync(d.dirty, 0, (size_t)g->h.n_points, static_cast<hipStream_t>(stream)));
        HIP_TRY(hipMemsetAsync(d.dirty_hdr + kDirtyHdrRejected, 0, sizeof(int32_t), static_cast<hipStream_t>(stream)));
    }
    d.all_dirty = all_dirty != 0;
    return NIN_OK;
}
```

ninpol_amd/csrc/device_grid.hpp:

```cpp
#pragma once
#include <cstdint>
#include <string>
#include <vector>

#include "gls_plan.hpp"

namespace nin {

struct GridView {
    int32_t n_points, n_elems, n_faces, dim;
    const int32_t *esup_ptr;
    const int32_t *esup;
    const int32_t *fsup_ptr;
    const int32_t *fsup;
    const double *coords;
    const double *centroids;
    const double *centroids4;
    const int32_t *face_cells;
    const double *face_center;
    const float *face_normal;
    const double *perm;
    const double *diff_mag;
    const uint8_t *flags;
};

NIN_HD inline int32_t gls_class_budget(int c) { return c == 0 ? 10240 : c == 1 ? 32768 : c == 2 ? 81920 : c == 3 ? 159744 : 0; }
NIN_HD inline int32_t gls_class_waves(int c) { return c == 0 ? 1 : c == 1 ? 2 : c == 2 ? 4 : c == 3 ? 8 : 1; }
NIN_HD inline int64_t gls_block_lds_bytes(int64_t ne, int64_t m, int64_t n, int waves) {
    const int64_t doubles = 2 + (n + 1) * (m | 1) + (waves == 1 ? 2 : (waves != 4 ? 2 : 1) * waves) * n + ((ne + 1) >> 1) +
                            ((ne + 7) >> 3);
    return ((doubles * 8 + 15) / 16) * 16;
}
NIN_HD inline int gls_node_class(int64_t ne, int64_t nf, int64_t nbf, bool force_global, int64_t *bytes, int64_t *rows,
                                 int64_t *cols) {
    const int64_t m = ne + 3 * (nf - nbf) + nbf, n = 3 * ne + 1;
    int c = kGlsClasses - 1;
    int64_t b = ((((ne + 1) >> 1) + n + m * n) * 8 + 15) / 16 * 16;
    for (int k = 0; k < kGlsClasses - 1 && !force_global && n <= 256; ++k) {
        const int64_t need = gls_block_lds_bytes(ne, m, n, gls_class_waves(k));
        if (need <= gls_class_budget(k)) { c = k; b = need; break; }
    }
    *bytes = b; *rows = m; *cols = n;
    return c;
}

struct DeviceGrid {
    int device = -1;
    GridView v{};
    int64_t nnz_e = 0, nnz_f = 0;
    bool fields_set = false, have_perm = false;
    bool prebuilt = false;
    std::vector<void *> allocs;

    static constexpr int kE2eChunks = 4;
    int32_t chunk_node[kE2eChunks + 1] = {0, 0, 0, 0, 0};
    bool chunkable = false;
    struct GlsList {
        int32_t count = 0;
        int32_t *nodes = nullptr;
        uint32_t *desc = nullptr;
        int32_t chunk_off[kE2eChunks + 1] = {};
        int32_t lds_bytes = 0;
        int32_t waves = 1;
        int32_t col_slots = 1;
        int32_t rows_per_lane = 1;
    } plan[kGlsPlanKernels];
    double *mfg_tiles = nullptr;
    int32_t mfg_slots = 0;
    const int32_t *noncube_nodes = nullptr;
    int32_t noncube_count = 0;
    bool noncube_nodes_ready = false;
    double *gls_scratch = nullptr;
    int64_t gls_scratch_stride = 0;
    int32_t gls_scratch_slots = 0;
    int32_t *gls_queue = nullptr;
    double *e2e_weights = nullptr, *e2e_nws = nullptr, *e2e_data = nullptr;
    int32_t *e2e_cnt = nullptr, *e2e_ptr = nullptr, *e2e_indices = nullptr;
    void *e2e_tmp = nullptr;
    size_t e2e_tmp_bytes = 0;
    double *apply_weights = nullptr;
    int32_t *tr_cell_ptr = nullptr, *tr_cell_pos = nullptr, *tr_cell_node = nullptr;
    struct AdjBin {
        int32_t count = 0;
        int32_t *nodes = nullptr;
        int64_t bytes = 0;
    } adj_bin[4];
    bool adj_ready = false;
    double *adj_contrib = nullptr, *adj_scratch = nullptr;
    int64_t adj_scratch_stride = 0;
    int32_t adj_scratch_slots = 0;
    double *shape_cell = nullptr, *shape_face = nullptr, *shape_slot = nullptr;
    double *shape_tan_cell = nullptr, *shape_tan_face = nullptr;
    int32_t shape_tan_n = 0;
    uint8_t *adj_node_bin = nullptr;
    int32_t *adj_dirty_lists = nullptr, *adj_dirty_hist = nullptr, *adj_dirty_hdr = nullptr;
    void *adj_dirty_tmp = nullptr;
    size_t adj_dirty_tmp_bytes = 0;
    int32_t *up_inpoel = nullptr, *up_inpofa = nullptr;
    int8_t *up_etype = nullptr;
    double *up_areas = nullptr;
    bool up_areas_valid = false;
    int64_t geom_updates = 0;
    void *ev_geom = nullptr;
    int64_t field_updates = 0;
    const uint8_t *node_class = nullptr;
    uint8_t *dirty = nullptr;
    int32_t *dirty_hdr = nullptr;
    bool all_dirty = true;
    bool scattered_cells = false, scattered_nodes = false, scattered_flags = false;
    bool scattered_marks = false;
    int64_t flag_updates = 0;
    bool flags_host_stale = false;
    int32_t *dirty_lists = nullptr, *dirty_hist = nullptr;
    void *dirty_tmp = nullptr;
    size_t dirty_tmp_bytes = 0;
    uint32_t *dirty_desc = nullptr;
    size_t dirty_desc_words = 0;
    uint8_t *flag_staging = nullptr;
    void *copy_stream = nullptr, *copy_stream2 = nullptr;
    void *ev_weights = nullptr, *ev_scan = nullptr;
    void *side_stream = nullptr, *ev_fork = nullptr, *ev_join = nullptr;
    bool side_pending = false;
    bool gls_too_large = false;
};

struct HostGrid;
int build_grid_on_device(HostGrid &h, DeviceGrid &d, int device, const int64_t *connectivity,
                         const int64_t *element_types, const double *xyz, int coords_dim, std::string *err);

}
```

ninpol_amd/csrc/fields_scatter.hip:

```cpp
#include <hip/hip_runtime.h>
#include <hipcub/hipcub.hpp>

#include <cstdint>

#include "diff_mag.hpp"
#include "launch.hpp"

namespace nin {

namespace {

constexpr int TPB = 256;
constexpr int WAVES = TPB / 64;
constexpr int NK = kGlsPlanKernels;
static_assert(TPB == 256, "the compaction fills its class-byte table with one thread per byte value");

inline unsigned blocks_for(int64_t n) { return (unsigned)((n + TPB - 1) / TPB); }

template <bool SCALED, class Id>
__global__ __launch_bounds__(TPB) void nin_scatter_perm_kernel(int64_t m, const Id *__restrict__ ids, const double *__restrict__ K,
                                                                const double *__restrict__ scale, int32_t E, int32_t P, uint64_t npoel8,
                                                                const int4 *__restrict__ inpoel, const int8_t *__restrict__ etype,
                                                                double *__restrict__ perm, double *__restrict__ diff_mag,
                                                                uint8_t *__restrict__ dirty, int32_t *__restrict__ rejected) {
    const int64_t i = (int64_t)blockIdx.x * TPB + threadIdx.x;
    if (i >= m) return;
    const int64_t e = (int64_t)ids[i];
    if (e < 0 || e >= (int64_t)E) {
        atomicAdd(rejected, 1);
        return;
    }
    double v[9];
#pragma unroll
    for (int k = 0; k < 9; ++k) v[k] = K[i * 9 + k];
    if (SCALED) {
        const double s = scale[i];
#pragma unroll
        for (int k = 0; k < 9; ++k) v[k] = s * v[k];
    }
#pragma unroll
    for (int k = 0; k < 9; ++k) perm[e * 9 + k] = v[k];
    diff_mag[e] = diff_mag_of(v[0], v[4], v[8]);
    const int4 a = inpoel[2 * e], b = inpoel[2 * e + 1];
    const int32_t q[8] = {a.x, a.y, a.z, a.w, b.x, b.y, b.z, b.w};
    const int n = (int)((npoel8 >> (8 * (etype[e] & 7))) & 0xff);
#pragma unroll
    for (int j = 0; j < 8; ++j)
        if (j < n && q[j] >= 0 && q[j] < P) dirty[q[j]] = 1;
}

template <bool FILL>
__global__ __launch_bounds__(TPB) void nin_dirty_compact_kernel(int32_t P, int32_t nblocks, int single, int clear, uint8_t *__restrict__ dirty,
                                                                 const uint8_t *__restrict__ cls, const int32_t *__restrict__ rejected,
                                                                 int32_t *__restrict__ hist, int32_t *__restrict__ lists,
                                                                 int32_t *__restrict__ hdr) {
    __shared__ int32_t wave_cnt[WAVES][NK];
    __shared__ int8_t kernel_of[256];
    const int tid = threadIdx.x, lane = tid & 63, w = tid >> 6;
    kernel_of[tid] = single ? (int8_t)0 : (int8_t)gls_class_kernel(tid);
    for (int i = tid; i < WAVES * NK; i += TPB) (&wave_cnt[0][0])[i] = 0;
    __syncthreads();
    const int64_t p = (int64_t)blockIdx.x * TPB + tid;
    bool has = p < P && dirty[p] != 0;
    const int key = has ? (int)kernel_of[cls[p]] : -1;
    has = has && key >= 0;
    int rank = 0;
    unsigned long long todo = __ballot(has);
    while (todo) {
        const int leader = __ffsll(todo) - 1;
        const int kk = __shfl(key, leader);
        const unsigned long long mk = __ballot(has && key == kk);
        if (has && key == kk) rank = __popcll(mk & ((1ull << lane) - 1ull));
        if (lane == leader) wave_cnt[w][kk] = __popcll(mk);
        todo &= ~mk;
    }
    __syncthreads();
    if (!FILL) {
        if (tid < NK) {
            int32_t c = 0;
            for (int ww = 0; ww < WAVES; ++ww) c += wave_cnt[ww][tid];
            hist[(int64_t)tid * nblocks + blockIdx.x] = c;
        }
        if (blockIdx.x == 0 && tid == NK) hist[(int64_t)NK * nblocks] = 0;
    } else {
        if (has) {
            int32_t at = hist[(int64_t)key * nblocks + blockIdx.x];
            for (int ww = 0; ww < w; ++ww) at += wave_cnt[ww][key];
            lists[at + rank] = (int32_t)p;
            if (clear && *rejected == 0) dirty[p] = 0;
        }
        if (blockIdx.x == 0 && tid <= NK) hdr[kDirtyHdrOffsets + tid] = hist[(int64_t)tid * nblocks];
    }
}

__global__ __launch_bounds__(TPB) void nin_dirty_count_kernel(int32_t P, const uint8_t *__restrict__ dirty, int32_t *__restrict__ out) {
    const int64_t p = (int64_t)blockIdx.x * TPB + threadIdx.x;
    const unsigned long long mk = __ballot(p < P && dirty[p] != 0);
    if ((threadIdx.x & 63) == 0 && mk) atomicAdd(out, (int32_t)__popcll(mk));
}

template <bool SCALED, class Id>
void scatter_variant(int64_t n, const void *ids, const double *K, const double *scale, const GridView &g, uint64_t npoel8, const int32_t *inpoel,
                     const int8_t *etype, uint8_t *dirty, int32_t *rejected, hipStream_t stream) {
    hipLaunchKernelGGL((nin_scatter_perm_kernel<SCALED, Id>), dim3(blocks_for(n)), dim3(TPB), 0, stream, n, static_cast<const Id *>(ids), K, scale,
                       g.n_elems, g.n_points, npoel8, reinterpret_cast<const int4 *>(inpoel), etype, const_cast<double *>(g.perm),
                       const_cast<double *>(g.diff_mag), dirty, rejected);
}

}

int launch_scatter_permeability(const GridView &g, uint64_t npoel8, const int32_t *inpoel, const int8_t *etype, const void *dev_ids,
                                int ids_are_int64, int64_t n, const double *dev_K, const double *dev_scale, uint8_t *dirty, int32_t *rejected,
                                hipStream_t stream) {
    if (n <= 0) return 0;
    if (n > (int64_t)INT32_MAX * TPB) return -5;
    if (dev_scale) {
        if (ids_are_int64) scatter_variant<true, int64_t>(n, dev_ids, dev_K, dev_scale, g, npoel8, inpoel, etype, dirty, rejected, stream);
        else scatter_variant<true, int32_t>(n, dev_ids, dev_K, dev_scale, g, npoel8, inpoel, etype, dirty, rejected, stream);
    } else {
        if (ids_are_int64) scatter_variant<false, int64_t>(n, dev_ids, dev_K, dev_scale, g, npoel8, inpoel, etype, dirty, rejected, stream);
        else scatter_variant<false, int32_t>(n, dev_ids, dev_K, dev_scale, g, npoel8, inpoel, etype, dirty, rejected, stream);
    }
    return hipGetLastError() == hipSuccess ? 0 : -3;
}

size_t dirty_compact_hist_ints(int32_t n_points) { return (size_t)NK * blocks_for(n_points) + 1; }

int dirty_compact_tmp_bytes(int32_t n_points, size_t *bytes) {
    *bytes = 0;
    int32_t *none = nullptr;
    return hipcub::DeviceScan::ExclusiveSum(nullptr, *bytes, none, none, (int)dirty_compact_hist_ints(n_points), nullptr) == hipSuccess ? 0 : -3;
}

int launch_dirty_compact(int32_t n_points, int single, int clear, uint8_t *dirty, const uint8_t *node_class, const int32_t *rejected,
                         int32_t *hist, int32_t *scanned, void *tmp, size_t tmp_bytes, int32_t *lists, int32_t *hdr, hipStream_t stream) {
    if (n_points <= 0) return 0;
    const int32_t nblocks = (int32_t)blocks_for(n_points);
    hipLaunchKernelGGL((nin_dirty_compact_kernel<false>), dim3(nblocks), dim3(TPB), 0, stream, n_points, nblocks, single, 0, dirty, node_class, rejected,
                       hist, lists, hdr);
    if (hipGetLastError() != hipSuccess) return -3;
    if (hipcub::DeviceScan::ExclusiveSum(tmp, tmp_bytes, hist, scanned, (int)dirty_compact_hist_ints(n_points), stream) != hipSuccess) return -3;
    hipLaunchKernelGGL((nin_dirty_compact_kernel<true>), dim3(nblocks), dim3(TPB), 0, stream, n_points, nblocks, single, clear, dirty, node_class, rejected,
                       scanned, lists, hdr);
    return hipGetLastError() == hipSuccess ? 0 : -3;
}

int launch_dirty_count(int32_t n_points, const uint8_t *dirty, int32_t *out, hipStream_t stream) {
    if (n_points <= 0) return 0;
    hipLaunchKernelGGL(nin_dirty_count_kernel, dim3(blocks_for(n_points)), dim3(TPB), 0, stream, n_points, dirty, out);
    return hipGetLastError() == hipSuccess ? 0 : -3;
}

}
```

ninpol_amd/csrc/gls_plan.hpp:

```cpp
#pragma once
#include <cstdint>

#ifdef __HIPCC__
#define NIN_HD __host__ __device__
#else
#define NIN_HD
#endif

namespace nin {

constexpr int kGlsClasses = 5;

constexpr int kGlsPlanKernels = 22;
namespace gk {
enum GlsKernel : int {
    block1, block2, block4, block8, scratch,
    hex8,
    mfw_large, mfw_small, mfw_general,
    small4, small8, small12,
    quad4,
    mfx_6x10, mfx_7x11, mfx_8x13, mfx_9x15, mfx_10x16,
    mfx_boundary,
    mfg_tiles,
    mfx_4x7,
    mfx_7x12,
};
}
using gk::GlsKernel;

enum class GlsFamily : uint8_t {
    block,
    scratch,
    hex8,
    mfw,
    small,
    quad4,
    mfx,
    mfg,
};

constexpr int kGlsQueueLine = 16;
constexpr int kGlsQueueHex8 = 0, kGlsQueueHex8Lines = 8;
constexpr int kGlsQueueBlock = 1;
constexpr int kGlsQueueMfw = 5;
constexpr int kGlsQueueMfx = 8, kGlsQueueMfxLists = 8;
constexpr int kGlsQueueMfg = 8 * kGlsQueueLine;
constexpr int kGlsQueueInts = 9 * kGlsQueueLine;
static_assert(kGlsQueueBlock > kGlsQueueHex8 && kGlsQueueBlock + (kGlsClasses - 1) <= kGlsQueueMfw, "block counters overlap");
static_assert(kGlsQueueMfw + 3 <= kGlsQueueMfx, "mfw counters overlap the mfx counters");
static_assert(kGlsQueueMfx + kGlsQueueMfxLists <= kGlsQueueLine, "the block / mfw / mfx counters must stay between hex8's ints 0 and 16");
static_assert(kGlsQueueMfg % kGlsQueueLine == 0 && kGlsQueueMfg / kGlsQueueLine >= kGlsQueueHex8 / kGlsQueueLine + kGlsQueueHex8Lines,
              "the mfg counter must lie on none of hex8's eight lines");
static_assert(kGlsQueueMfg < kGlsQueueInts, "the mfg counter lies outside the block");

struct GlsPlanRow {
    GlsFamily family;
    int8_t sub;
    uint8_t class_byte;
    int16_t desc_words;
    int16_t fdq_word;
    int16_t counter;
};
constexpr int kGlsDescHex8 = 32, kGlsDescQuad4 = 2, kGlsDescMfw = 40, kGlsDescMfx = 56, kGlsDescMfg = 124;

NIN_HD constexpr GlsPlanRow gls_plan_row(int k) {
    using F = GlsFamily;
    constexpr GlsPlanRow rows[kGlsPlanKernels] = {
        {F::block,   0,    0,  0,             -1,  kGlsQueueBlock + 0},
        {F::block,   1,    1,  0,             -1,  kGlsQueueBlock + 1},
        {F::block,   2,    2,  0,             -1,  kGlsQueueBlock + 2},
        {F::block,   3,    3,  0,             -1,  kGlsQueueBlock + 3},
        {F::scratch, 4,    4,  0,             -1,  -1},
        {F::hex8,    0,  255,  kGlsDescHex8,  -1,  kGlsQueueHex8},
        {F::mfw,     0,  254,  kGlsDescMfw,   24,  kGlsQueueMfw + 0},
        {F::mfw,     1,  253,  kGlsDescMfw,   24,  kGlsQueueMfw + 1},
        {F::mfw,     2,  252,  kGlsDescMfw,   24,  kGlsQueueMfw + 2},
        {F::small,   0,  249,  0,             -1,  -1},
        {F::small,   1,  250,  0,             -1,  -1},
        {F::small,   2,  251,  0,             -1,  -1},
        {F::quad4,   0,  248,  kGlsDescQuad4, -1,  -1},
        {F::mfx,     0,  243,  kGlsDescMfx,    0,  kGlsQueueMfx + 0},
        {F::mfx,     1,  244,  kGlsDescMfx,    0,  kGlsQueueMfx + 1},
        {F::mfx,     2,  245,  kGlsDescMfx,    0,  kGlsQueueMfx + 2},
        {F::mfx,     3,  246,  kGlsDescMfx,    0,  kGlsQueueMfx + 3},
        {F::mfx,     4,  247,  kGlsDescMfx,    0,  kGlsQueueMfx + 4},
        {F::mfx,     5,  242,  kGlsDescMfx,    0,  kGlsQueueMfx + 5},
        {F::mfg,     0,  241,  kGlsDescMfg,    0,  kGlsQueueMfg},
        {F::mfx,     6,  240,  kGlsDescMfx,    0,  kGlsQueueMfx + 6},
        {F::mfx,     7,  239,  kGlsDescMfx,    0,  kGlsQueueMfx + 7},
    };
    return rows[k];
}

NIN_HD constexpr uint8_t gls_class_byte(GlsKernel k) { return gls_plan_row(k).class_byte; }
NIN_HD constexpr int gls_class_kernel(int class_byte) {
    for (int k = 0; k < kGlsPlanKernels; ++k)
        if (gls_plan_row(k).class_byte == class_byte) return k;
    return -1;
}

enum GlsRoute : int {
    kRouteHex8 = 1,
    kRouteMfw = 2,
    kRouteMfwGeneral = 4,
    kRouteSmall = 8,
    kRouteQuad4 = 16,
    kRouteMfx = 32,
    kRouteMfxTakesGeneral = 64,
    kRouteMfxNoBoundary = 128,
    kRouteMfg = 256,
    kRouteMfxSmall = 512,
    kRouteMfx7x12 = 1024,
};

static_assert(gk::block1 == 0 && gk::scratch == 4 && gk::hex8 == 5 && gk::mfw_large == 6 && gk::mfw_general == 8 && gk::small4 == 9 &&
                  gk::small12 == 11 && gk::quad4 == 12 && gk::mfx_6x10 == 13 && gk::mfx_10x16 == 17 && gk::mfx_boundary == 18 &&
                  gk::mfg_tiles == 19 && gk::mfx_4x7 == 20 && gk::mfx_7x12 == 21 && gk::mfx_7x12 + 1 == kGlsPlanKernels,
              "GlsKernel must keep the public numbering of include/ninpol_amd.h");
constexpr bool plan_class_bytes_ok() {
    for (int k = 0; k < kGlsPlanKernels; ++k) {
        const GlsPlanRow r = gls_plan_row(k);
        const bool sized = r.family == GlsFamily::block || r.family == GlsFamily::scratch;
        if (sized != (k < kGlsClasses) || (sized && (r.class_byte != k || r.sub != k)) || (!sized && r.class_byte < kGlsClasses)) return false;
        for (int j = 0; j < k; ++j)
            if (gls_plan_row(j).class_byte == r.class_byte) return false;
    }
    for (int i = 0; i < 5; ++i)
        if (gls_class_byte(GlsKernel(gk::mfx_6x10 + i)) != gls_class_byte(gk::mfx_6x10) + i || gls_plan_row(gk::mfx_6x10 + i).sub != i) return false;
    return true;
}
constexpr bool plan_takes_int(int k, int i) {
    const GlsPlanRow r = gls_plan_row(k);
    if (r.counter < 0 || r.family != GlsFamily::hex8) return r.counter >= 0 && i == r.counter;
    return i >= r.counter && (i - r.counter) % kGlsQueueLine == 0 && (i - r.counter) / kGlsQueueLine < kGlsQueueHex8Lines;
}
constexpr bool plan_counters_ok() {
    for (int k = 0; k < kGlsPlanKernels; ++k) {
        const GlsPlanRow a = gls_plan_row(k);
        if (a.counter + (a.family == GlsFamily::hex8 ? kGlsQueueHex8Lines - 1 : 0) * kGlsQueueLine >= kGlsQueueInts) return false;
        for (int j = 0; j < kGlsPlanKernels; ++j)
            if (j != k && a.counter >= 0 && plan_takes_int(j, a.counter)) return false;
    }
    return true;
}
static_assert(plan_class_bytes_ok(), "class bytes: 0 .. 4 for the block / scratch classes, distinct and above 4 for every other kernel, mfx_6x10 .. mfx_10x16 in a row");
static_assert(plan_counters_ok(), "two kernels of the plan share a work counter, or one lies outside gls_queue");

}
```

ninpol_amd/csrc/launch.hpp:

```cpp
#pragma once
#include <hip/hip_runtime.h>

#include <cstdint>

#include "device_grid.hpp"

namespace nin {

#ifdef __HIPCC__
template <auto KERN>
inline int allow_dynamic_lds(size_t bytes) {
    if (bytes <= 48 * 1024) return 0;
    static size_t allowed[64] = {};
    int dev = 0;
    (void)hipGetDevice(&dev);
    size_t &a = allowed[dev & 63];
    if (bytes > a) {
        if (hipFuncSetAttribute(reinterpret_cast<const void *>(KERN), hipFuncAttributeMaxDynamicSharedMemorySize, (int)bytes) != hipSuccess) return -3;
        a = bytes;
    }
    return 0;
}
#endif

int launch_idw(const GridView &g, const int32_t *targets, int32_t n_targets, int32_t mx_row, int64_t nnz, double *out, double *nws,
               hipStream_t stream);
int launch_ls(const GridView &g, const int32_t *targets, int32_t n_targets, int32_t mx_row, int64_t nnz, double *out, double *nws,
              hipStream_t stream);
int launch_gls_class(const GridView &g, const int32_t *nodes, int32_t count, int32_t lds_bytes,
                     int32_t rows_per_lane, int add_neumann, double *out, double *nws,
                     double *scratch, int64_t scratch_stride, int32_t scratch_slots, hipStream_t stream);
int launch_gls_block(const GridView &g, const int32_t *nodes, int32_t count, int32_t waves, int32_t col_slots,
                     int32_t lds_bytes, int add_neumann, double *out, double *nws, int32_t *queue, hipStream_t stream);
const char *kernel_name_gls_block();
int launch_hex8_desc(const GridView &g, const int32_t *nodes, int32_t count, int32_t *desc, hipStream_t stream);
int launch_gls_hex8mf(const GridView &g, const int32_t *nodes, const int32_t *desc, int32_t count, int add_neumann,
                      double *out, double *nws, int32_t *queue, hipStream_t stream);
int launch_gls_hex8mf_apply(const GridView &g, const int32_t *nodes, const int32_t *desc, int32_t count, int add_neumann,
                            const double *u_cells, int32_t n_fields, double *values, double *nws, int32_t *queue, hipStream_t stream);
const char *kernel_name_gls_hex8mf();
int launch_mfw_desc(const GridView &g, const int32_t *nodes, int32_t count, uint32_t *desc, hipStream_t stream);
int launch_gls_mfw(const GridView &g, const int32_t *nodes, const uint32_t *desc, int32_t count, int kind, int add_neumann,
                   double *out, double *nws, int32_t *queue, hipStream_t stream);
const char *kernel_name_gls_mfw();
int launch_mfx_desc(const GridView &g, const int32_t *nodes, int32_t count, uint32_t *desc, hipStream_t stream);
int launch_gls_mfx(const GridView &g, const int32_t *nodes, const uint32_t *desc, int32_t count, int cls, int add_neumann, double *out,
                   double *nws, int32_t *queue, hipStream_t stream);
const char *kernel_name_gls_mfx();
int launch_mfg_desc(const GridView &g, const int32_t *nodes, int32_t count, uint32_t *desc, hipStream_t stream);
int launch_gls_mfg(const GridView &g, const int32_t *nodes, const uint32_t *desc, int32_t count, int add_neumann, double *out, double *nws,
                   int32_t *queue, double *tiles, int32_t n_slots, hipStream_t stream);
const char *kernel_name_gls_mfg();
int launch_quad4_desc(const GridView &g, const int32_t *nodes, int32_t count, int32_t *desc, hipStream_t stream);
int launch_gls_quad4(const GridView &g, const int32_t *nodes, const int32_t *desc, int32_t count, int add_neumann, double *out,
                     double *nws, hipStream_t stream);
int launch_gls_small(const GridView &g, const int32_t *nodes, int32_t count, int kind, int add_neumann, double *out, double *nws,
                     hipStream_t stream);

int launch_row_nnz(const GridView &g, const double *data, int32_t *row_nnz, hipStream_t stream, int32_t p_begin = 0, int32_t p_end = -1);
int launch_compact(const GridView &g, const double *data, const int32_t *new_ptr, int32_t *indices,
                   double *vals, hipStream_t stream, int32_t p_begin = 0, int32_t p_end = -1);
int launch_rows_range(const GridView &g, int method_ls, int32_t n_points, int32_t p_begin, int32_t p_end, int32_t mx_row, int64_t nnz,
                      double *out, double *nws, hipStream_t stream);

int launch_apply(const GridView &g, const double *data, const double *u, double *values, int32_t mx_row, int64_t nnz, hipStream_t stream);
int launch_apply_list(const GridView &g, const double *data, const double *u, int32_t k, double *values, const int32_t *list,
                      int32_t count, hipStream_t stream);
int launch_apply_fields(const GridView &g, const double *data, const double *u, int32_t k, double *values, int32_t mx_row, int64_t nnz,
                        hipStream_t stream);

int launch_apply_transpose(const GridView &g, const int32_t *cell_ptr, const int32_t *cell_pos, const int32_t *cell_node, int32_t mx_cell,
                           const double *data, const double *v, int32_t k, double *x, hipStream_t stream);
int launch_iota(int32_t *dst, int32_t n, hipStream_t stream);
int launch_transpose_index_fill(const GridView &g, const int32_t *sorted_cells, int32_t nnz, int32_t *cell_ptr, const int32_t *cell_pos,
                                int32_t *cell_node, hipStream_t stream);

int launch_sddmm(const GridView &g, const double *u, const double *v, int32_t k, double *grad, hipStream_t stream);

struct AdjBinRun {
    const int32_t *nodes;
    int32_t count;
    int64_t bytes;
    double *scratch;
    int64_t scratch_stride;
    int32_t scratch_slots;
};
int launch_adjoint_bytes(const GridView &g, int64_t *bytes, hipStream_t stream);
int launch_gls_adjoint(const GridView &g, int bin, const AdjBinRun &run, int add_neumann, const double *grad_csr, const double *grad_nws,
                       double *contrib, hipStream_t stream);
int launch_adjoint_gather(const GridView &g, const int32_t *cell_ptr, const int32_t *cell_pos, const double *contrib, double *grad_perm,
                          double *grad_diff_mag, hipStream_t stream);
struct AdjointReduce {
    int32_t n_params;
    const double *basis;
    int64_t stride;
};
int launch_gls_adjoint_reduced(const GridView &g, int bin, const AdjBinRun &run, int add_neumann, const double *grad_csr,
                               const double *grad_nws, const AdjointReduce &red, double *reduced, hipStream_t stream);
int launch_gls_adjoint_points(const GridView &g, int bin, const AdjBinRun &run, int add_neumann, const double *grad_csr,
                              const double *grad_nws, double *cell_bar, double *face_bar, double *own_bar, hipStream_t stream);
int launch_shape_gather(const GridView &g, const int32_t *inpofa, const int32_t *cell_ptr, const int32_t *cell_pos, double *cell_bar,
                        const double *face_bar, double *face_slot, double *grad_points, hipStream_t stream);
int launch_gls_tangent(const GridView &g, int bin, const AdjBinRun &run, int add_neumann, int32_t n_tangents, const double *tangent_perm,
                       const double *tangent_diff_mag, double *tangent_csr, double *tangent_nws, int64_t nnz, hipStream_t stream);
int launch_shape_tangent_geometry(const GridView &g, const int32_t *inpoel, const int32_t *inpofa, int32_t n_tangents, const double *tangent_points,
                                  double *tangent_cell, double *tangent_face, hipStream_t stream);
int launch_gls_tangent_points(const GridView &g, int bin, const AdjBinRun &run, int add_neumann, int32_t n_tangents, const double *tangent_points,
                              const double *tangent_cell, const double *tangent_face, double *tangent_csr, double *tangent_nws, int64_t nnz,
                              hipStream_t stream);

int launch_jac_seed(const GridView &g, int64_t nnz, const double *u, double *grad_csr, hipStream_t stream);
int launch_jac_fold(const GridView &g, double *fold, hipStream_t stream);
int launch_jac_apply(const GridView &g, const double *contrib, const double *fold, int32_t n, const double *dperm, const double *ddm,
                     double *out, hipStream_t stream);
int launch_jac_apply_transpose(const GridView &g, const int32_t *cell_ptr, const int32_t *cell_pos, const int32_t *cell_node,
                               const double *contrib, const double *fold, int32_t n, const double *v, double *grad_perm, double *grad_dm,
                               hipStream_t stream);

int launch_jacr_apply(const GridView &g, int32_t M, const double *R, int32_t n, const double *dtheta, double *out, hipStream_t stream);
int launch_jacr_apply_transpose(const GridView &g, int32_t M, const int32_t *cell_ptr, const int32_t *cell_pos, const int32_t *cell_node,
                                const double *R, int32_t n, const double *v, double *grad_theta, hipStream_t stream);

constexpr int kXjacApplyChunk = 4, kXjacTransposeChunk = 2;
int launch_xjac_apply(const GridView &g, const int32_t *inpoel, const int32_t *inpofa, const double *cell_bar, const double *face_bar,
                      const double *own_bar, int32_t n, const double *dX, double *tangent_cell, double *tangent_face, double *out,
                      hipStream_t stream);
int launch_xjac_apply_transpose(const GridView &g, const int32_t *inpofa, const int32_t *cell_ptr, const int32_t *cell_pos,
                                const int32_t *cell_node, const double *cell_bar, const double *face_bar, const double *own_bar, int32_t n,
                                const double *v, double *cell_share, double *face_slot, double *grad_points, hipStream_t stream);

int launch_xjac_pattern_count(const GridView &g, const int32_t *inpoel, const int32_t *inpofa, int force_slow, int64_t *count, hipStream_t stream);
int xjac_pattern_scan(void *tmp, size_t *tmp_bytes, const int64_t *count, int64_t *block_ptr, int32_t n_points, hipStream_t stream);
int launch_xjac_pattern_fill(const GridView &g, const int32_t *inpoel, const int32_t *inpofa, int force_slow, const int64_t *block_ptr,
                             int32_t *block_col, hipStream_t stream);
int launch_xjac_assemble(const GridView &g, const int32_t *inpoel, const int32_t *inpofa, const double *cell_bar, const double *face_bar,
                         const double *own_bar, const int64_t *block_ptr, const int32_t *block_col, double *values, hipStream_t stream);

int launch_pad_centroids(const double *src, int64_t n_elems, double *dst, hipStream_t stream);
int launch_classify(const GridView &g, int use_group, int force_global, uint8_t *node_class,
                    unsigned long long *class_max, hipStream_t stream);

int launch_update_coords(const double *dev_xyz, int coords_dim, int64_t n_points, double *coords, hipStream_t stream);
int launch_update_geometry(const GridView &g, uint64_t npoel8, const int32_t *inpoel, const int8_t *etype, const int32_t *inpofa,
                           double *centroids, double *face_center, float *face_normal, double *face_area, hipStream_t stream);

hipError_t launch_update_permeability(int32_t n_elems, const double *dev_K, const double *dev_scale, double *perm, double *diff_mag,
                                      hipStream_t stream);

constexpr int kDirtyHdrOffsets = 0, kDirtyHdrRejected = kGlsPlanKernels + 2, kDirtyHdrCount = kGlsPlanKernels + 3, kDirtyHdrInts = 32;
static_assert(kDirtyHdrCount < kDirtyHdrInts, "the dirty set's header block is too small for the plan");
int launch_scatter_permeability(const GridView &g, uint64_t npoel8, const int32_t *inpoel, const int8_t *etype, const void *dev_ids,
                                int ids_are_int64, int64_t n, const double *dev_K, const double *dev_scale, uint8_t *dirty, int32_t *rejected,
                                hipStream_t stream);
int launch_scatter_points(const GridView &g, uint64_t npoel8, const int32_t *inpoel, const int8_t *etype, const int32_t *inpofa,
                          const void *dev_ids, int ids_are_int64, int64_t n, const double *dev_xyz, int coords_dim, double *face_area,
                          uint8_t *dirty, int32_t *rejected, hipStream_t stream);
int launch_set_flags(int32_t n_points, const void *dev_flags, int flags_are_bytes, uint8_t *flags, uint8_t *dirty, hipStream_t stream);
int launch_scatter_flags(int32_t n_points, const void *dev_ids, int ids_are_int64, int64_t n, const void *dev_flags, int flags_are_bytes,
                         uint8_t *flags, uint8_t *dirty, int32_t *rejected, hipStream_t stream);
size_t dirty_compact_hist_ints(int32_t n_points);
int dirty_compact_tmp_bytes(int32_t n_points, size_t *bytes);
int launch_dirty_compact(int32_t n_points, int single, int clear, uint8_t *dirty, const uint8_t *node_class, const int32_t *rejected,
                         int32_t *hist, int32_t *scanned, void *tmp, size_t tmp_bytes, int32_t *lists, int32_t *hdr, hipStream_t stream);
int launch_dirty_count(int32_t n_points, const uint8_t *dirty, int32_t *out, hipStream_t stream);

int launch_dirty_row_nnz(const GridView &g, const double *data, const int32_t *list, int32_t total, int32_t *pack_cnt, int32_t *cnt,
                         int32_t *changed, hipStream_t stream);
int launch_dirty_pack(const GridView &g, const double *data, const double *nws, const int32_t *list, int32_t total, const int32_t *pack_off,
                      int32_t *pack_node, double *pack_nws, int32_t *pack_indices, double *pack_data, hipStream_t stream);

constexpr int kAdjDirtyHdrInts = 8;
int launch_adj_bin_byte(const int32_t *nodes, int32_t count, int32_t n_points, int bin, uint8_t *bin_of, hipStream_t stream);
size_t adj_dirty_hist_ints(int32_t n_points);
int adj_dirty_tmp_bytes(int32_t n_points, size_t *bytes);
int launch_adj_dirty_compact(int32_t n_points, int clear, uint8_t *dirty, const uint8_t *bin_of, const int32_t *rejected, int32_t *hist,
                             int32_t *scanned, void *tmp, size_t tmp_bytes, int32_t *lists, int32_t *hdr, hipStream_t stream);
int launch_jac_seed_rows(const GridView &g, const int32_t *list, int32_t total, const double *u, double *grad_csr, hipStream_t stream);
int launch_mark_dirty(const GridView &g, uint64_t npoel8, const int32_t *inpoel, const int8_t *etype, const void *dev_ids, int ids_are_int64,
                      int64_t n, int ids_are_cells, uint8_t *dirty, int32_t *rejected, hipStream_t stream);

const char *kernel_name_idw();
const char *kernel_name_ls();
const char *kernel_name_gls();

}
```

ninpol_amd/grid.py:

```python
import ctypes
import warnings

import numpy as np

from . import _lib
from . import topology as T
from ._args import is_torch, on_gpu

_SCALARS = ("dim", "n_elems", "n_points", "n_faces", "n_edges", "MX_ELEMENTS_PER_POINT",
            "MX_POINTS_PER_POINT", "MX_ELEMENTS_PER_FACE", "MX_FACES_PER_POINT")
_SHAPES = {"esuel": T.MAX_FACES_PER_ELEMENT, "infael": T.MAX_FACES_PER_ELEMENT, "inpofa": T.MAX_POINTS_PER_FACE,
           "inpoel": T.MAX_POINTS_PER_ELEMENT, "inedel": T.MAX_EDGES_PER_ELEMENT, "inpoed": 2,
           "centroids": 3, "faces_centers": 3, "normal_faces": 3, "point_coords": 3}
_ARRAYS = ("esup", "esup_ptr", "psup", "psup_ptr", "fsup", "fsup_ptr", "esuf", "esuf_ptr", "esuel", "infael",
           "inpofa", "inpoel", "inpoed", "inedel", "boundary_faces", "boundary_points", "point_coords",
           "centroids", "faces_centers", "normal_faces", "faces_areas", "element_types")


def _ptr(a):
    return a.ctypes.data_as(ctypes.c_void_p)


def _dev_ptr(t):
    return None if t is None else ctypes.c_void_p(t.data_ptr())


def _dev_ids(t):
    return ctypes.c_void_p(t.data_ptr()), int(t.element_size() == 8), int(t.numel())


def _stream_of(t):
    import torch
    return ctypes.c_void_p(torch.cuda.current_stream(t.device).cuda_stream)


class _PlanCounts(dict):

    def __missing__(self, key):
        if key == "mfx":
            return sum(v for k, v in self.items() if k.startswith("mfx_") and k != "mfx_boundary")
        raise KeyError(key)


class Grid:

    def __init__(self, dim, n_elems, n_points, npoel, nfael, lnofa, lpofa, nedel, lpoed, connectivity,
                 element_types, logging=False, build_edges=False, coords=None, num_threads=0, build_device=None):
        if dim < 1:
            raise ValueError("The number of dimensions must be greater than 0.")
        if n_elems < 1:
            raise ValueError("The number of elements must be greater than 0.")
        if n_points < 1:
            raise ValueError("The number of points must be greater than 0.")
        i64 = lambda a: np.ascontiguousarray(a, dtype=np.int64)
        tabs = [i64(npoel), i64(nfael), i64(lnofa), i64(lpofa), i64(nedel), i64(lpoed)]
        expected = [(T.NUM_ELEMENT_TYPES,), (T.NUM_ELEMENT_TYPES,),
                    (T.NUM_ELEMENT_TYPES, T.MAX_FACES_PER_ELEMENT),
                    (T.NUM_ELEMENT_TYPES, T.MAX_FACES_PER_ELEMENT, T.MAX_POINTS_PER_FACE),
                    (T.NUM_ELEMENT_TYPES,), (T.NUM_ELEMENT_TYPES, T.MAX_EDGES_PER_ELEMENT, T.MAX_POINTS_PER_EDGE)]
        for a, shp in zip(tabs, expected):
            if a.shape != shp:
                raise ValueError(f"The array must have shape {shp}, not {a.shape}.")
        conn = i64(connectivity)
        if conn.shape != (n_elems, T.MAX_POINTS_PER_ELEMENT):
            raise ValueError(f"The array must have shape {(n_elems, T.MAX_POINTS_PER_ELEMENT)}, not {conn.shape}.")
        etypes = i64(element_types)
        if coords is None:
            raise ValueError("The point coordinates have not been set.")
        xyz = np.ascontiguousarray(coords, dtype=np.float64)
        if xyz.ndim != 2 or xyz.shape[0] != n_points or not 1 <= xyz.shape[1] <= 3:
            raise ValueError(f"coords must have shape ({n_points}, 1..3), not {xyz.shape}.")
        self.logging = bool(logging)
        self.build_edges = bool(build_edges)
        self._cache = {}
        self._no_fields_resident()
        self._h = ctypes.c_void_p()
        L = _lib.load()
        if build_device is None:
            rc = L.nin_grid_create(int(dim), int(n_elems), int(n_points), *[_ptr(a) for a in tabs], _ptr(conn),
                                   _ptr(etypes), _ptr(xyz), int(xyz.shape[1]), int(bool(build_edges)),
                                   int(num_threads), ctypes.byref(self._h))
        else:
            rc = L.nin_grid_create_on_device(int(dim), int(n_elems), int(n_points), *[_ptr(a) for a in tabs], _ptr(conn),
                                             _ptr(etypes), _ptr(xyz), int(xyz.shape[1]), int(bool(build_edges)),
                                             int(build_device), ctypes.byref(self._h))
        if rc == _lib.NIN_EINVAL:
            raise ValueError(L.nin_last_error().decode())
        _lib.check(rc)
        self._coords_dim = int(xyz.shape[1])
        self.are_elements_loaded = True
        self.are_coords_loaded = True
        self.are_structures_built = True
        self.are_centroids_calculated = True
        self.are_normals_calculated = True

    def __del__(self):
        h = getattr(self, "_h", None)
        if h:
            try:
                _lib.load().nin_grid_destroy(h)
            except Exception:
                pass
            self._h = None

    def build(self):
        return None

    def load_point_coords(self, coords=None):
        if coords is None:
            return None
        L = _lib.load()
        shape = (int(self.n_points), self._coords_dim)
        if on_gpu(coords):
            import torch
            if tuple(coords.shape) != shape:
                raise ValueError(f"points must have shape {shape}, not {tuple(coords.shape)}.")
            if coords.dtype != torch.float64:
                raise ValueError(f"points on the device must be float64, not {coords.dtype}.")
            if self.device < 0 or coords.device.index != self.device:
                raise ValueError(f"points are on {coords.device}, the grid is on " +
                                 (f"cuda:{self.device}" if self.device >= 0 else "no device (call to_device first)") + ".")
            t = coords.detach().contiguous()
            rc = L.nin_grid_update_points_device(self._h, _dev_ptr(t), self._coords_dim, _stream_of(t))
        else:
            if is_torch(coords):
                coords = coords.detach().numpy()
            try:
                xyz = np.ascontiguousarray(coords, dtype=np.float64)
            except (TypeError, ValueError) as e:
                raise ValueError(f"points cannot be converted to float64: {e}") from e
            if xyz.shape != shape:
                raise ValueError(f"points must have shape {shape}, not {xyz.shape}.")
            rc = L.nin_grid_update_points(self._h, _ptr(xyz), self._coords_dim)
        self._points_moved(rc)
        return None

    def _points_moved(self, rc):
        for name in ("point_coords", "centroids", "faces_centers", "normal_faces", "faces_areas"):
            self._cache.pop(name, None)
        if rc == _lib.NIN_EINVAL:
            raise ValueError(_lib.load().nin_last_error().decode())
        _lib.check(rc)

    def scatter_point_coords(self, nodes, rows):
        L = _lib.load()
        if is_torch(rows):
            rc = L.nin_grid_scatter_points_device(self._h, *_dev_ids(nodes), _dev_ptr(rows), self._coords_dim, _stream_of(rows))
        else:
            rc = L.nin_grid_scatter_points(self._h, _ptr(nodes), int(len(nodes)), _ptr(rows), self._coords_dim)
        self._points_moved(rc)

    def calculate_centroids(self):
        return None

    def calculate_normal_faces(self):
        return None

    def _scalar(self, name):
        return int(_lib.load().nin_grid_scalar(self._h, name.encode()))

    def _array(self, name):
        if name in self._cache:
            return self._cache[name]
        L = _lib.load()
        n, dt = ctypes.c_int64(), ctypes.c_int()
        _lib.check(L.nin_grid_array_info(self._h, name.encode(), ctypes.byref(n), ctypes.byref(dt)))
        a = np.empty(n.value, dtype=np.float64 if dt.value == 1 else np.int64)
        _lib.check(L.nin_grid_array_copy(self._h, name.encode(), _ptr(a), n.value))
        if name in _SHAPES:
            a = a.reshape(-1, _SHAPES[name])
            if name == "point_coords" and self._coords_dim != 3:
                a = np.ascontiguousarray(a[:, :self._coords_dim])
        self._cache[name] = a
        return a

    @property
    def nnz_esup(self):
        return self._scalar("nnz_esup")

    def __getattr__(self, name):
        if name in _SCALARS:
            return self._scalar(name)
        if name in _ARRAYS:
            return self._array(name)
        raise AttributeError(name)

    def get_data(self):
        if not self.build_edges:
            raise ValueError("Invalid shape in axis 0: 0.")
        data = {k: getattr(self, k) for k in ("n_elems", "n_points", "n_faces", "n_edges", "MX_ELEMENTS_PER_POINT",
                                              "MX_POINTS_PER_POINT", "MX_ELEMENTS_PER_FACE", "MX_FACES_PER_POINT")}
        for k in ("point_coords", "centroids", "normal_faces", "faces_centers", "faces_areas", "boundary_faces",
                  "boundary_points", "inpoel", "element_types", "inpofa", "infael", "inpoed", "inedel"):
            data[k] = getattr(self, k).copy()

        def dense(ptr, idx, n_rows, width):
            out = -np.ones((n_rows, width), dtype=np.int64)
            cnt = np.diff(ptr)
            rows = np.repeat(np.arange(n_rows), cnt)
            cols = np.arange(len(idx)) - np.repeat(ptr[:-1], cnt)
            out[rows, cols] = idx
            return out
        data["esup"] = dense(self.esup_ptr, self.esup, self.n_points, self.MX_ELEMENTS_PER_POINT)
        data["psup"] = dense(self.psup_ptr, self.psup, self.n_points, self.MX_POINTS_PER_POINT)
        data["esuf"] = dense(self.esuf_ptr, self.esuf, self.n_faces, self.MX_ELEMENTS_PER_FACE)
        data["fsup"] = dense(self.fsup_ptr, self.fsup, self.n_points, self.MX_FACES_PER_POINT)
        return data

    def to_device(self, device=0):
        self._no_fields_resident()
        _lib.check(_lib.load().nin_grid_to_device(self._h, int(device)))
        return self

    def _no_fields_resident(self):
        self._perm_key = self._fields_variable = self._flags_key = None
        self._perm_from_device = self._flags_from_device = self._perm_edited_last_call = False

    def host_permeability_resident(self, key):
        self._perm_key, self._perm_from_device = key, False

    def host_permeability_edited(self):
        self._perm_from_device = False

    def permeability_from_device(self, fingerprint, *host_rows):
        if self._perm_key is None:
            self._perm_key = fingerprint(*host_rows)
        self._perm_from_device = True

    def permeability_edit_seen(self, edited):
        self._perm_edited_last_call = edited

    def host_flags_uploaded(self, variable):
        if self._flags_from_device or self._fields_variable not in (None, variable):
            self.mark_all_dirty()
        self._fields_variable, self._flags_from_device, self._flags_key = variable, False, None

    def flags_from_device(self, variable, fingerprint, host_row):
        if not (self._flags_from_device and self._fields_variable == variable and self._flags_key is not None):
            self._flags_key = fingerprint(host_row)
        self._fields_variable, self._flags_from_device = variable, True

    def flags_fetched(self):
        self._flags_from_device, self._flags_key = False, None

    def load_permeability_device(self, K, scale=None):
        _lib.check(_lib.load().nin_fields_set_permeability_device(self._h, _dev_ptr(K), _dev_ptr(scale), _stream_of(K)))

    def scatter_permeability_device(self, cells, K, scale=None):
        _lib.check(_lib.load().nin_fields_scatter_permeability_device(self._h, *_dev_ids(cells), _dev_ptr(K), _dev_ptr(scale), _stream_of(K)))

    def load_flags_device(self, flags):
        _lib.check(_lib.load().nin_fields_set_flags_device(self._h, _dev_ptr(flags), int(flags.element_size() == 1), _stream_of(flags)))

    def scatter_flags_device(self, nodes, flags):
        _lib.check(_lib.load().nin_fields_scatter_flags_device(self._h, *_dev_ids(nodes), _dev_ptr(flags), int(flags.element_size() == 1), _stream_of(flags)))

    def fetch_flags(self):
        if self.device < 0:
            return None
        out = np.empty(int(self.n_points), dtype=np.uint8)
        rc = _lib.load().nin_fields_get_flags(self._h, _ptr(out))
        if rc == _lib.NIN_ESTATE:
            return None
        _lib.check(rc)
        return out

    @property
    def flag_updates(self):
        return int(_lib.load().nin_grid_flag_updates(self._h))

    @property
    def dirty_nodes(self):
        n = int(_lib.load().nin_grid_dirty_nodes(self._h))
        if n < -1:
            _lib.check(_lib.NIN_EHIP)
        return n

    def clear_dirty(self, stream=0):
        _lib.check(_lib.load().nin_grid_dirty_reset(self._h, 0, ctypes.c_void_p(stream)))

    def mark_all_dirty(self, stream=0):
        _lib.check(_lib.load().nin_grid_dirty_reset(self._h, 1, ctypes.c_void_p(stream)))

    def mark_dirty(self, cells=None, nodes=None, stream=0):
        from . import _args
        if (cells is None) == (nodes is None):
            raise ValueError("mark_dirty takes exactly one of cells= and nodes=")
        ids, name, n = (cells, "cells", self.n_elems) if nodes is None else (nodes, "nodes", self.n_points)
        L = _lib.load()
        if self.device < 0:
            _lib.check(L.nin_grid_mark_dirty_device(self._h, None, 0, 0, int(nodes is None), None))
        import torch
        on_host = not on_gpu(ids)
        if on_host:
            ids = torch.from_numpy(_args.host_ids(_args.to_host(ids), name, int(n))).to(torch.device("cuda", self.device))
        else:
            _args.device_ids(ids, name, self.device)
            ids = ids.detach().contiguous()
        s = ctypes.c_void_p(stream) if stream and not on_host else _stream_of(ids)
        _lib.check(L.nin_grid_mark_dirty_device(self._h, *_dev_ids(ids), int(nodes is None), s))
        if on_host:
            torch.cuda.current_stream(ids.device).synchronize()

    def fetch_permeability(self):
        if self.device < 0:
            return None
        E = int(self.n_elems)
        perm, dmag = np.empty((E, 9), dtype=np.float64), np.empty(E, dtype=np.float64)
        rc = _lib.load().nin_fields_get_permeability(self._h, _ptr(perm), _ptr(dmag))
        if rc == _lib.NIN_ESTATE:
            return None
        _lib.check(rc)
        return perm, dmag

    @property
    def field_updates(self):
        return int(_lib.load().nin_grid_field_updates(self._h))

    @property
    def device(self):
        return int(_lib.load().nin_grid_device(self._h))

    @property
    def geometry_updates(self):
        return int(_lib.load().nin_grid_geometry_updates(self._h))

    @property
    def has_transpose_index(self):
        return bool(_lib.load().nin_grid_has_transpose_index(self._h))

    def release_scratch(self):
        _lib.check(_lib.load().nin_grid_release_scratch(self._h))

    ADJOINT_BINS = ("lds1", "lds2", "lds4", "global")

    def gls_adjoint_plan(self):
        counts = np.zeros(4, dtype=np.int64)
        _lib.check(_lib.load().nin_gls_adjoint_plan(self._h, counts.ctypes.data_as(ctypes.c_void_p)))
        return dict(zip(self.ADJOINT_BINS, counts.tolist()))

    PLAN_KERNELS = ("block1", "block2", "block4", "block8", "scratch", "hex8", "mfw_large", "mfw_small", "mfw_general", "small4", "small8",
                    "small12", "quad4", "mfx_6x10", "mfx_7x11", "mfx_8x13", "mfx_9x15", "mfx_10x16", "mfx_boundary", "mfg_tiles", "mfx_4x7", "mfx_7x12")

    def gls_plan_flops(self):
        alg, ref, comp = np.zeros(22), np.zeros(22), np.zeros(22, dtype=np.int64)
        p = lambda a: a.ctypes.data_as(ctypes.c_void_p)
        _lib.check(_lib.load().nin_gls_plan_flops(self._h, p(alg), p(ref), p(comp)))
        return {k: (float(alg[i]), float(ref[i]), int(comp[i])) for i, k in enumerate(self.PLAN_KERNELS)}

    def gls_plan(self):
        counts = np.zeros(22, dtype=np.int64)
        _lib.check(_lib.load().nin_gls_plan(self._h, counts.ctypes.data_as(ctypes.c_void_p)))
        return _PlanCounts(zip(self.PLAN_KERNELS, counts.tolist()))
```

Baseline: 2291.

## Add specialised prism6 GLS kernel for fixed-stencil mfw_small nodes

Splits the mfw_small plan list into generic nodes and nodes whose descriptor matches a fixed prism-like stencil (a fixed face and neighbour count, each neighbour seen three times), and sends the latter to a new kernel. That kernel unrolls the local least-squares factor and solve for this fixed shape using wave-level LDS staging. The aim is to drop the general-case overhead of the mfw kernel for a common node pattern. The split adds a new class byte, an extra list and queue counter, and host-side reordering, all of which must stay consistent across the dirty-update and side-stream paths. On a pure hex mesh few nodes may match.

```diff
diff --git a/include/ninpol_amd.h b/include/ninpol_amd.h
--- a/include/ninpol_amd.h
+++ b/include/ninpol_amd.h
@@ -220,6 +220,8 @@
 
 int nin_gls_plan(const nin_grid *g, int64_t counts[22]);
 
+int nin_gls_prism6_nodes(const nin_grid *g, int64_t *count, uint8_t *mask);
+
 int nin_gls_plan_flops(nin_grid *g, double alg[22], double ref[22], int64_t computed[22]);
 
 #define NIN_EXCHANGE_HANDLE_BYTES 64
diff --git a/ninpol_amd/_lib.py b/ninpol_amd/_lib.py
--- a/ninpol_amd/_lib.py
+++ b/ninpol_amd/_lib.py
@@ -14,7 +14,7 @@
     "nin_fields_set", "nin_weights_device", "nin_weights_host", "nin_csr_compact_host", "nin_interpolate_csr_host", "nin_apply_host",
     "nin_apply_device", "nin_apply_fields_host", "nin_spmv_device", "nin_spmv_transpose_device", "nin_apply_transpose_fields_host",
     "nin_pack_connectivity", "nin_pack_table_row", "nin_diff_mag",
-    "nin_algorithmic_bytes", "nin_kernel_name", "nin_gls_plan", "nin_gls_plan_flops", "nin_host_alloc", "nin_host_free", "nin_hash64",
+    "nin_algorithmic_bytes", "nin_kernel_name", "nin_gls_plan", "nin_gls_prism6_nodes", "nin_gls_plan_flops", "nin_host_alloc", "nin_host_free", "nin_hash64",
     "nin_grid_release_scratch",
     "nin_grid_update_points", "nin_grid_update_points_device", "nin_grid_geometry_updates", "nin_grid_has_transpose_index",
     "nin_fields_set_permeability_device", "nin_fields_get_permeability", "nin_grid_field_updates",
@@ -154,6 +154,8 @@
     L.nin_kernel_name.argtypes = [i32]
     L.nin_kernel_name.restype = cp
     L.nin_gls_plan.argtypes = [vp, vp]
+    if hasattr(L, "nin_gls_prism6_nodes"):
+        L.nin_gls_prism6_nodes.argtypes = [vp, ctypes.POINTER(i64), vp]
     L.nin_gls_plan_flops.argtypes = [vp, vp, vp, vp]
     L.nin_host_alloc.argtypes = [ctypes.c_size_t, ctypes.POINTER(vp)]
     L.nin_host_free.argtypes = [vp]
diff --git a/ninpol_amd/build.py b/ninpol_amd/build.py
--- a/ninpol_amd/build.py
+++ b/ninpol_amd/build.py
@@ -18,6 +18,7 @@
     ("kernels_gls_block.hip", "hipcc", []),
     ("kernels_gls_hex8mf.hip", "hipcc", ["-mllvm", "-amdgpu-atomic-optimizer-strategy=None"]),
     ("kernels_gls_mfw.hip", "hipcc", []),
+    ("kernels_gls_prism6.hip", "hipcc", []),
     ("kernels_gls_mfx.hip", "hipcc", []),
     ("kernels_gls_mfg.hip", "hipcc", []),
     ("kernels_gls_quad4.hip", "hipcc", []),
diff --git a/ninpol_amd/csrc/abi_plan.hip b/ninpol_amd/csrc/abi_plan.hip
--- a/ninpol_amd/csrc/abi_plan.hip
+++ b/ninpol_amd/csrc/abi_plan.hip
@@ -122,6 +122,49 @@
         case GlsFamily::mfg: return launch_gls_mfg(d.v, nodes, desc, count, add_neumann, out, nws, queue, d.mfg_tiles, d.mfg_slots, stream);
     }
     return NIN_EINVAL;
+}
+
+int launch_mfw_small(const DeviceGrid &d, const int32_t *nodes_rest, const uint32_t *desc_rest, int32_t n_rest, const int32_t *nodes_p6,
+                     const uint32_t *desc_p6, int32_t n_p6, int add_neumann, double *out, double *nws, hipStream_t stream) {
+    const GlsPlanRow r = gls_plan_row(gk::mfw_small);
+    int rc = 0;
+    if (n_rest > 0) rc = launch_gls_mfw(d.v, nodes_rest, desc_rest, n_rest, r.sub, add_neumann, out, nws, d.gls_queue + r.counter, stream);
+    if (rc || n_p6 <= 0) return rc;
+    if (getenv("NIN_GLS_NO_PRISM6") != nullptr || getenv("NIN_MFW_LANE_COLUMNS") != nullptr || getenv("NIN_MFW_SMALL_STRIPS") != nullptr)
+        return launch_gls_mfw(d.v, nodes_p6, desc_p6, n_p6, r.sub, add_neumann, out, nws, d.gls_queue + kGlsQueuePrism6, stream);
+    return launch_gls_prism6(d.v, nodes_p6, desc_p6, n_p6, add_neumann, out, nws, d.gls_queue + kGlsQueuePrism6, stream);
+}
+
+int split_prism6(nin_grid *g, const std::vector<int32_t> &list) {
+    DeviceGrid &d = g->d;
+    auto &l = d.plan[gk::mfw_small];
+    constexpr int K = DeviceGrid::kE2eChunks;
+    l.p6_count = 0;
+    for (int j = 0; j <= K; ++j) l.p6_chunk_off[j] = 0;
+    if (!l.count) return NIN_OK;
+    std::vector<uint8_t> flags((size_t)l.count);
+    {
+        DevTmp<uint8_t> df;
+        if (hipMalloc((void **)&df, (size_t)l.count) != hipSuccess) return fail(NIN_ENOMEM, "hipMalloc");
+        if (launch_prism6_flags(l.desc, l.count, df, nullptr) || hipMemcpy(flags.data(), df, (size_t)l.count, hipMemcpyDeviceToHost) != hipSuccess)
+            return fail(NIN_EHIP, "prism6 selection: %s", hipGetErrorString(hipGetLastError()));
+    }
+    std::vector<int32_t> rest, p6;
+    for (int32_t i = 0; i < l.count; ++i) (flags[i] ? p6 : rest).push_back(list[i]);
+    if (p6.empty()) return NIN_OK;
+    for (int32_t p : p6) g->node_class[p] = (uint8_t)kGlsPrism6Byte;
+    if (hipMemcpy(const_cast<uint8_t *>(d.node_class), g->node_class.data(), g->node_class.size(), hipMemcpyHostToDevice) != hipSuccess)
+        return fail(NIN_EHIP, "prism6 selection: uploading the class bytes");
+    l.p6_count = (int32_t)p6.size();
+    for (int j = 0; j <= K; ++j) {
+        l.chunk_off[j] = (int32_t)(std::lower_bound(rest.begin(), rest.end(), d.chunk_node[j]) - rest.begin());
+        l.p6_chunk_off[j] = (int32_t)(std::lower_bound(p6.begin(), p6.end(), d.chunk_node[j]) - p6.begin());
+    }
+    rest.insert(rest.end(), p6.begin(), p6.end());
+    if (hipMemcpy(l.nodes, rest.data(), rest.size() * 4, hipMemcpyHostToDevice) != hipSuccess) return fail(NIN_EHIP, "prism6 selection: uploading the list");
+    if (launch_plan_desc(d, gk::mfw_small, l.nodes, l.count, l.desc, nullptr) || hipDeviceSynchronize() != hipSuccess)
+        return fail(NIN_EHIP, "descriptor kernel of plan kernel %d", (int)gk::mfw_small);
+    return NIN_OK;
 }
 
 }
@@ -197,6 +240,7 @@
             if ((rc = dev_alloc(d, &l.desc, (size_t)l.count * words))) return rc;
             if (launch_plan_desc(d, GlsKernel(k), l.nodes, l.count, l.desc, nullptr)) return fail(NIN_EHIP, "descriptor kernel of plan kernel %d", k);
         }
+        if (k == gk::mfw_small && (rc = split_prism6(g, lists[k]))) return rc;
     }
     if (d.plan[gk::mfg_tiles].count) {
         d.mfg_slots = std::min<int32_t>(d.plan[gk::mfg_tiles].count, kMfgResidentWaves);
@@ -232,8 +276,14 @@
 struct PlanRange { const int32_t *nodes; const uint32_t *desc; int32_t count; };
 static PlanRange plan_range(const DeviceGrid &d, GlsKernel k, int piece) {
     const auto &l = d.plan[k];
-    const int32_t b = piece < 0 ? 0 : l.chunk_off[piece], n = (piece < 0 ? l.count : l.chunk_off[piece + 1]) - b;
+    const int32_t b = piece < 0 ? 0 : l.chunk_off[piece], n = (piece < 0 ? l.count - l.p6_count : l.chunk_off[piece + 1]) - b;
     return {l.nodes ? l.nodes + b : nullptr, l.desc ? l.desc + (size_t)gls_plan_row(k).desc_words * b : nullptr, n};
+}
+static PlanRange plan_range_prism6(const DeviceGrid &d, int piece) {
+    const auto &l = d.plan[gk::mfw_small];
+    const int32_t first = l.count - l.p6_count;
+    const int32_t b = first + (piece < 0 ? 0 : l.p6_chunk_off[piece]), n = first + (piece < 0 ? l.p6_count : l.p6_chunk_off[piece + 1]) - b;
+    return {l.nodes ? l.nodes + b : nullptr, l.desc ? l.desc + (size_t)gls_plan_row(gk::mfw_small).desc_words * b : nullptr, n};
 }
 
 int nin::gls_side_begin(DeviceGrid &d, int piece, int add_neumann, double *out, double *nws, hipStream_t stream) {
@@ -270,6 +320,11 @@
     for (GlsKernel k : kMainOrder) {
         if ((k == gk::hex8 && !cube) || (only >= 0 && only != k) || (d.side_pending && on_side_stream(k))) continue;
         const PlanRange r = plan_range(d, k, piece);
+        if (k == gk::mfw_small) {
+            const PlanRange r6 = plan_range_prism6(d, piece);
+            if (!rc) rc = launch_mfw_small(d, r.nodes, r.desc, r.count, r6.nodes, r6.desc, r6.count, add_neumann, out, nws, stream);
+            continue;
+        }
         if (!rc && r.count > 0) rc = launch_plan_kernel(d, k, r.nodes, r.desc, r.count, add_neumann, out, nws, stream);
     }
     if (!rc) rc = gls_side_end(d, stream);
@@ -281,20 +336,26 @@
     const bool gls = method == NIN_METHOD_GLS;
     if (laps) laps->mark(1);
     if (gls) {
-        for (int k = 0; k < kGlsPlanKernels; ++k)
-            if (launch_plan_desc(d, GlsKernel(k), lists + off[k], off[k + 1] - off[k], desc + desc_first[k], stream))
-                return fail(NIN_EHIP, "descriptor kernel of plan kernel %d", k);
+        for (int k = 0; k < kGlsLists; ++k)
+            if (launch_plan_desc(d, k == kGlsListPrism6 ? gk::mfw_small : GlsKernel(k), lists + off[k], off[k + 1] - off[k], desc + desc_first[k], stream))
+                return fail(NIN_EHIP, "descriptor kernel of list %d", k);
         HIP_TRY(hipMemsetAsync(d.gls_queue, 0, kGlsQueueInts * sizeof(int32_t), stream));
     }
     if (laps) laps->mark(2);
     int rc = 0;
     if (!gls)
-        rc = method == NIN_METHOD_IDW ? launch_idw(d.v, lists, off[kGlsPlanKernels], 0, 0, out, nws, stream)
-                                      : launch_ls(d.v, lists, off[kGlsPlanKernels], 0, 0, out, nws, stream);
+        rc = method == NIN_METHOD_IDW ? launch_idw(d.v, lists, off[kGlsLists], 0, 0, out, nws, stream)
+                                      : launch_ls(d.v, lists, off[kGlsLists], 0, 0, out, nws, stream);
     else
-        for (GlsKernel k : kMainOrder)
-            if (!rc && off[k + 1] > off[k])
-                rc = launch_plan_kernel(d, k, lists + off[k], desc + desc_first[k], off[k + 1] - off[k], add_neumann, out, nws, stream);
+        for (GlsKernel k : kMainOrder) {
+            if (rc) break;
+            const int32_t n = off[k + 1] - off[k];
+            if (k == gk::mfw_small)
+                rc = launch_mfw_small(d, lists + off[k], desc + desc_first[k], n, lists + off[kGlsListPrism6], desc + desc_first[kGlsListPrism6],
+                                      off[kGlsListPrism6 + 1] - off[kGlsListPrism6], add_neumann, out, nws, stream);
+            else if (n > 0)
+                rc = launch_plan_kernel(d, k, lists + off[k], desc + desc_first[k], n, add_neumann, out, nws, stream);
+        }
     if (rc) return fail(rc, "kernel launch failed: %s", hipGetErrorString(hipGetLastError()));
     if (laps) laps->mark(3);
     return NIN_OK;
@@ -330,18 +391,18 @@
     HIP_TRY(hipMemsetAsync(dev_neumann_ws, 0, (size_t)P * 8, stream));
     if (n_targets == 0) return NIN_OK;
     const bool gls = method == NIN_METHOD_GLS;
-    std::vector<int32_t> lists[kGlsPlanKernels];
-    for (int64_t i = 0; i < n_targets; ++i) lists[gls ? gls_class_kernel(g->node_class[targets[i]]) : 0].push_back((int32_t)targets[i]);
+    std::vector<int32_t> lists[kGlsLists];
+    for (int64_t i = 0; i < n_targets; ++i) lists[gls ? gls_class_list(g->node_class[targets[i]]) : 0].push_back((int32_t)targets[i]);
     std::vector<int32_t> flat;
-    int32_t off[kGlsPlanKernels + 1];
-    size_t desc_first[kGlsPlanKernels], words = 0;
-    for (int k = 0; k < kGlsPlanKernels; ++k) {
+    int32_t off[kGlsLists + 1];
+    size_t desc_first[kGlsLists], words = 0;
+    for (int k = 0; k < kGlsLists; ++k) {
         off[k] = (int32_t)flat.size();
         desc_first[k] = words = desc_align(words);
         flat.insert(flat.end(), lists[k].begin(), lists[k].end());
-        if (gls) words += lists[k].size() * (size_t)gls_plan_row(k).desc_words;
-    }
-    off[kGlsPlanKernels] = (int32_t)flat.size();
+        if (gls) words += lists[k].size() * (size_t)gls_plan_row(k == kGlsListPrism6 ? (int)gk::mfw_small : k).desc_words;
+    }
+    off[kGlsLists] = (int32_t)flat.size();
     const size_t list_words = desc_align(flat.size());
     DevTmp<int32_t> dl0;
     HIP_TRY(hipMalloc((void **)&dl0, (list_words + words) * 4));
@@ -483,6 +544,15 @@
     return NIN_OK;
 }
 
+int nin_gls_prism6_nodes(const nin_grid *g, int64_t *count, uint8_t *mask) {
+    if (!g || !count) return fail(NIN_EINVAL, "NULL argument");
+    if (int rc = on_device(g, kHintToDevice)) return rc;
+    *count = g->d.plan[gk::mfw_small].p6_count;
+    if (mask)
+        for (int64_t p = 0; p < g->h.n_points; ++p) mask[p] = g->node_class[p] == kGlsPrism6Byte;
+    return NIN_OK;
+}
+
 int nin_gls_plan(const nin_grid *g, int64_t counts[22]) {
     if (!g || !counts) return fail(NIN_EINVAL, "NULL argument");
     if (int rc = on_device(g, kHintToDevice)) return rc;
diff --git a/ninpol_amd/csrc/abi_update.hip b/ninpol_amd/csrc/abi_update.hip
--- a/ninpol_amd/csrc/abi_update.hip
+++ b/ninpol_amd/csrc/abi_update.hip
@@ -409,15 +409,15 @@
         return NIN_OK;
     }
     const int32_t *off = hdr + kDirtyHdrOffsets;
-    const int32_t total = off[kGlsPlanKernels];
+    const int32_t total = off[kGlsLists];
     if (total < 0 || total > P) return fail(NIN_EHIP, "the dirty set's lists hold %d nodes of %d", (int)total, (int)P);
     if (n_recomputed) *n_recomputed = total;
     if (total == 0) return NIN_OK;
-    size_t desc_first[kGlsPlanKernels], words = 0;
-    for (int k = 0; gls && k < kGlsPlanKernels; ++k) {
+    size_t desc_first[kGlsLists], words = 0;
+    for (int k = 0; gls && k < kGlsLists; ++k) {
         if (off[k + 1] < off[k]) return fail(NIN_EHIP, "the dirty set's lists are out of order");
         desc_first[k] = words = desc_align(words);
-        words += (size_t)(off[k + 1] - off[k]) * (size_t)gls_plan_row(k).desc_words;
+        words += (size_t)(off[k + 1] - off[k]) * (size_t)gls_plan_row(k == kGlsListPrism6 ? (int)gk::mfw_small : k).desc_words;
     }
     if (words > d.dirty_desc_words && (rc = grow(d, &d.dirty_desc, &d.dirty_desc_words, words + words / 2))) return rc;
     if ((rc = launch_lists(d, method, d.dirty_lists, off, d.dirty_desc, desc_first, add_neumann, dev_csr_data, dev_neumann_ws, stream, &laps)))
diff --git a/ninpol_amd/csrc/device_grid.hpp b/ninpol_amd/csrc/device_grid.hpp
--- a/ninpol_amd/csrc/device_grid.hpp
+++ b/ninpol_amd/csrc/device_grid.hpp
@@ -60,6 +60,8 @@
         int32_t *nodes = nullptr;
         uint32_t *desc = nullptr;
         int32_t chunk_off[kE2eChunks + 1] = {};
+        int32_t p6_count = 0;
+        int32_t p6_chunk_off[kE2eChunks + 1] = {};
         int32_t lds_bytes = 0;
         int32_t waves = 1;
         int32_t col_slots = 1;
diff --git a/ninpol_amd/csrc/fields_scatter.hip b/ninpol_amd/csrc/fields_scatter.hip
--- a/ninpol_amd/csrc/fields_scatter.hip
+++ b/ninpol_amd/csrc/fields_scatter.hip
@@ -12,7 +12,8 @@
 
 constexpr int TPB = 256;
 constexpr int WAVES = TPB / 64;
-constexpr int NK = kGlsPlanKernels;
+constexpr int NK = kGlsLists;
+static_assert(kDirtyHdrOffsets + NK < kDirtyHdrRejected, "the lists' offsets run into the header's other words");
 static_assert(TPB == 256, "the compaction fills its class-byte table with one thread per byte value");
 
 inline unsigned blocks_for(int64_t n) { return (unsigned)((n + TPB - 1) / TPB); }
@@ -57,7 +58,7 @@
     __shared__ int32_t wave_cnt[WAVES][NK];
     __shared__ int8_t kernel_of[256];
     const int tid = threadIdx.x, lane = tid & 63, w = tid >> 6;
-    kernel_of[tid] = single ? (int8_t)0 : (int8_t)gls_class_kernel(tid);
+    kernel_of[tid] = single ? (int8_t)0 : (int8_t)gls_class_list(tid);
     for (int i = tid; i < WAVES * NK; i += TPB) (&wave_cnt[0][0])[i] = 0;
     __syncthreads();
     const int64_t p = (int64_t)blockIdx.x * TPB + tid;
diff --git a/ninpol_amd/csrc/gls_plan.hpp b/ninpol_amd/csrc/gls_plan.hpp
--- a/ninpol_amd/csrc/gls_plan.hpp
+++ b/ninpol_amd/csrc/gls_plan.hpp
@@ -45,13 +45,16 @@
 constexpr int kGlsQueueMfw = 5;
 constexpr int kGlsQueueMfx = 8, kGlsQueueMfxLists = 8;
 constexpr int kGlsQueueMfg = 8 * kGlsQueueLine;
-constexpr int kGlsQueueInts = 9 * kGlsQueueLine;
+constexpr int kGlsQueuePrism6 = 9 * kGlsQueueLine;
+constexpr int kGlsQueueInts = 10 * kGlsQueueLine;
 static_assert(kGlsQueueBlock > kGlsQueueHex8 && kGlsQueueBlock + (kGlsClasses - 1) <= kGlsQueueMfw, "block counters overlap");
 static_assert(kGlsQueueMfw + 3 <= kGlsQueueMfx, "mfw counters overlap the mfx counters");
 static_assert(kGlsQueueMfx + kGlsQueueMfxLists <= kGlsQueueLine, "the block / mfw / mfx counters must stay between hex8's ints 0 and 16");
 static_assert(kGlsQueueMfg % kGlsQueueLine == 0 && kGlsQueueMfg / kGlsQueueLine >= kGlsQueueHex8 / kGlsQueueLine + kGlsQueueHex8Lines,
               "the mfg counter must lie on none of hex8's eight lines");
 static_assert(kGlsQueueMfg < kGlsQueueInts, "the mfg counter lies outside the block");
+static_assert(kGlsQueuePrism6 % kGlsQueueLine == 0 && kGlsQueuePrism6 > kGlsQueueMfg && kGlsQueuePrism6 < kGlsQueueInts,
+              "the prism6 counter must lie on a line of its own inside the block");
 
 struct GlsPlanRow {
     GlsFamily family;
@@ -92,12 +95,16 @@
     return rows[k];
 }
 
+constexpr int kGlsPrism6Byte = 238;
+constexpr int kGlsLists = kGlsPlanKernels + 1, kGlsListPrism6 = kGlsPlanKernels;
+
 NIN_HD constexpr uint8_t gls_class_byte(GlsKernel k) { return gls_plan_row(k).class_byte; }
 NIN_HD constexpr int gls_class_kernel(int class_byte) {
     for (int k = 0; k < kGlsPlanKernels; ++k)
         if (gls_plan_row(k).class_byte == class_byte) return k;
-    return -1;
+    return class_byte == kGlsPrism6Byte ? (int)gk::mfw_small : -1;
 }
+NIN_HD constexpr int gls_class_list(int class_byte) { return class_byte == kGlsPrism6Byte ? kGlsListPrism6 : gls_class_kernel(class_byte); }
 
 enum GlsRoute : int {
     kRouteHex8 = 1,
@@ -120,6 +127,7 @@
 constexpr bool plan_class_bytes_ok() {
     for (int k = 0; k < kGlsPlanKernels; ++k) {
         const GlsPlanRow r = gls_plan_row(k);
+        if (r.class_byte == kGlsPrism6Byte) return false;
         const bool sized = r.family == GlsFamily::block || r.family == GlsFamily::scratch;
         if (sized != (k < kGlsClasses) || (sized && (r.class_byte != k || r.sub != k)) || (!sized && r.class_byte < kGlsClasses)) return false;
         for (int j = 0; j < k; ++j)
@@ -138,6 +146,7 @@
     for (int k = 0; k < kGlsPlanKernels; ++k) {
         const GlsPlanRow a = gls_plan_row(k);
         if (a.counter + (a.family == GlsFamily::hex8 ? kGlsQueueHex8Lines - 1 : 0) * kGlsQueueLine >= kGlsQueueInts) return false;
+        if (plan_takes_int(k, kGlsQueuePrism6)) return false;
         for (int j = 0; j < kGlsPlanKernels; ++j)
             if (j != k && a.counter >= 0 && plan_takes_int(j, a.counter)) return false;
     }
diff --git a/ninpol_amd/csrc/kernels_gls_prism6.hip b/ninpol_amd/csrc/kernels_gls_prism6.hip
--- /dev/null
+++ b/ninpol_amd/csrc/kernels_gls_prism6.hip
@@ -0,0 +1,293 @@
+#include <hip/hip_runtime.h>
+
+#include <cstdlib>
+#include <utility>
+
+#include "device_grid.hpp"
+#include "gls_device_math.hpp"
+#include "launch.hpp"
+#include "mfw_desc.hpp"
+#include "mfw_strips.hpp"
+
+namespace nin {
+
+namespace {
+
+using namespace glsmath;
+using mfwstrips::row_allsum;
+
+constexpr int P6_F = 6, P6_D = 6, P6_NC = 3 * P6_D, P6_SLOTS = 3;
+constexpr int P6_STAGE_F = 70;
+constexpr int P6_LDS_D = P6_F * P6_STAGE_F, P6_LDS_Y = P6_LDS_D + 3 * P6_D, P6_LDS_W = P6_LDS_Y + P6_NC, P6_LDS_Z = P6_LDS_W + P6_F + P6_D,
+              P6_NODE_DOUBLES = (P6_LDS_Z + 3 + 1) & ~1;
+static_assert(7 * P6_F + P6_D == 16 * P6_SLOTS, "the dense problem's rows fill three slots of 16 lanes");
+static_assert(2 * 8 * (16 * P6_NODE_DOUBLES + TAU_TAB_DOUBLES) <= 160 * 1024, "two workgroups per CU");
+
+template <int L>
+__device__ __forceinline__ double row_bcast(double v) { return dpp_mov<0x150 + L>(v); }
+
+template <int T>
+__device__ __forceinline__ void p6_step(double (&C)[P6_SLOTS][P6_NC + 1], double (&rinv)[2], int r) {
+    constexpr int KT = T / 16, LT = T % 16;
+    const bool piv = r == LT;
+    double x[P6_SLOTS], ss = 0.0;
+#pragma unroll
+    for (int k = KT; k < P6_SLOTS; ++k) {
+        x[k] = (k == KT && r <= LT) ? 0.0 : C[k][T];
+        ss = fma(x[k], x[k], ss);
+    }
+    const House h = house_unguarded(row_bcast<LT>(C[KT][T]), row_allsum(ss));
+    x[KT] = piv ? h.vp : x[KT];
+    rinv[KT] = piv ? h.rinv : rinv[KT];
+#pragma unroll
+    for (int j = T + 1; j <= P6_NC; ++j) {
+        double d = x[KT] * C[KT][j];
+#pragma unroll
+        for (int k = KT + 1; k < P6_SLOTS; ++k) d = fma(x[k], C[k][j], d);
+        const double w = -(h.g * row_allsum(d));
+#pragma unroll
+        for (int k = KT; k < P6_SLOTS; ++k) C[k][j] = fma(w, x[k], C[k][j]);
+    }
+    C[KT][T] = piv ? h.beta : C[KT][T];
+}
+template <int... T>
+__device__ __forceinline__ void p6_factor(double (&C)[P6_SLOTS][P6_NC + 1], double (&rinv)[2], int r, std::integer_sequence<int, T...>) {
+    (p6_step<T>(C, rinv, r), ...);
+}
+
+template <int K>
+__device__ __forceinline__ void p6_back(const double (&C)[P6_SLOTS][P6_NC + 1], const double (&rinv)[2], double (&ct)[2], double (&y)[2], int r) {
+    constexpr int KT = K / 16, LT = K % 16;
+    const double yk = row_bcast<LT>(ct[KT] * rinv[KT]);
+    y[KT] = r == LT ? yk : y[KT];
+    ct[0] = (K >= 16 || r < K) ? fma(-yk, C[0][K], ct[0]) : ct[0];
+    if (K > 16) ct[1] = 16 + r < K ? fma(-yk, C[1][K], ct[1]) : ct[1];
+}
+template <int... I>
+__device__ __forceinline__ void p6_solve(const double (&C)[P6_SLOTS][P6_NC + 1], const double (&rinv)[2], double (&ct)[2], double (&y)[2], int r,
+                                         std::integer_sequence<int, I...>) {
+    (p6_back<P6_NC - 1 - I>(C, rinv, ct, y, r), ...);
+}
+
+__global__ __launch_bounds__(256, 2) void nin_gls_prism6_kernel(GridView g, const int32_t *__restrict__ nodes, const uint32_t *__restrict__ desc,
+                                                                int32_t count, int add_neumann, double *__restrict__ out,
+                                                                double *__restrict__ nws, int32_t *__restrict__ queue) {
+    __shared__ double lds_all[16][P6_NODE_DOUBLES];
+    __shared__ double tau_tab[TAU_TAB_DOUBLES];
+    tau_table_to_lds(tau_tab);
+    __syncthreads();
+    const lds_cdouble_ptr tau_lds = (lds_cdouble_ptr)tau_tab;
+    const int lane = threadIdx.x & 63;
+    if ((lane & 15) < 3) lds_all[threadIdx.x >> 4][P6_LDS_Z + (lane & 15)] = 0.0;
+    const int32_t n_groups = (count + 3) >> 2;
+    auto ticket = [&]() -> int32_t {
+        int32_t v = 0;
+        if (lane == 0) v = atomicAdd(queue, 1);
+        return __builtin_amdgcn_readfirstlane(v);
+    };
+    for (int32_t grp = ticket(); grp < n_groups; grp = ticket()) {
+        int ln;
+        asm volatile("v_mov_b32 %0, %1" : "=v"(ln) : "v"(threadIdx.x));
+        const int r = ln & 15;
+        double *const Nm = lds_all[ln >> 4];
+        double *const dbuf = Nm + P6_LDS_D, *const yb = Nm + P6_LDS_Y, *const wbuf = Nm + P6_LDS_W;
+        const bool p1 = r < 2 * P6_F;
+        const int f = p1 ? r >> 1 : 0, h = r & 1;
+        int32_t idx = 4 * grp + ((ln >> 4) & 3);
+        const bool valid = idx < count;
+        idx = valid ? idx : count - 1;
+        const int32_t p = nodes ? nodes[idx] : idx;
+        const uint32_t *dw = desc + (size_t)kMfwDescWords * idx;
+        const uint32_t w0 = dw[f], w1 = dw[12 + f];
+        const uint32_t eb = (uint32_t)g.esup_ptr[p], fb = (uint32_t)g.fsup_ptr[p];
+        const bool is_neu = (g.flags[p] & 2) != 0;
+        const double xv0 = g.coords[3 * (size_t)p + 0], xv1 = g.coords[3 * (size_t)p + 1], xv2 = g.coords[3 * (size_t)p + 2];
+        const uint32_t pe = w0 & 31;
+        const uint32_t po = (dw[r < P6_D ? r : 0] >> 21) & 31;
+        const uint32_t frec[3] = {(w0 >> 5) & 0xFFFFu, w1 & 0xFFFFu, w1 >> 16};
+        const uint32_t recA = h ? frec[1] : frec[0];
+
+        double uA[3], uB[3], dod[3];
+        {
+            const uint32_t ce = (uint32_t)g.esup[eb + pe], co = (uint32_t)g.esup[eb + po];
+            const uint32_t cA = (uint32_t)g.esup[eb + ((recA >> 11) & 31)], cB = (uint32_t)g.esup[eb + ((frec[2] >> 11) & 31)];
+            double P[10][3], BA[10][3], BB[10][3], de[3];
+            double Ke[9], KA[9], KB[9];
+#pragma unroll
+            for (int k = 0; k < 9; ++k) { Ke[k] = g.perm[9 * (size_t)ce + k]; KA[k] = g.perm[9 * (size_t)cA + k]; KB[k] = g.perm[9 * (size_t)cB + k]; }
+            const double dme = g.diff_mag[ce];
+            de[0] = g.centroids[3 * (size_t)ce + 0] - xv0;
+            de[1] = g.centroids[3 * (size_t)ce + 1] - xv1;
+            de[2] = g.centroids[3 * (size_t)ce + 2] - xv2;
+            dod[0] = g.centroids[3 * (size_t)co + 0] - xv0;
+            dod[1] = g.centroids[3 * (size_t)co + 1] - xv1;
+            dod[2] = g.centroids[3 * (size_t)co + 2] - xv2;
+#pragma unroll
+            for (int q = 0; q < 10; ++q) {
+#pragma unroll
+                for (int t = 0; t < 3; ++t) { BA[q][t] = 0.0; BB[q][t] = 0.0; }
+            }
+#pragma unroll
+            for (int t = 0; t < 3; ++t) P[0][t] = de[t];
+            BB[0][0] = h ? 0.0 : 1.0;
+#pragma unroll
+            for (int i = 0; i < 3; ++i) {
+                const uint32_t fc = (uint32_t)g.fsup[fb + (frec[i] & 63)];
+                const uint32_t cn = (uint32_t)g.esup[eb + ((frec[i] >> 11) & 31)];
+                const double N0 = (double)g.face_normal[3 * (size_t)fc + 0], N1 = (double)g.face_normal[3 * (size_t)fc + 1],
+                             N2 = (double)g.face_normal[3 * (size_t)fc + 2];
+                const double T0 = xv0 - g.face_center[3 * (size_t)fc + 0], T1 = xv1 - g.face_center[3 * (size_t)fc + 1],
+                             T2 = xv2 - g.face_center[3 * (size_t)fc + 2];
+                const double U0 = N1 * T2 - N2 * T1, U1 = N2 * T0 - N0 * T2, U2 = N0 * T1 - N1 * T0;
+                const double dmn = g.diff_mag[cn];
+                double eta = 0.0;
+                eta = dme > eta ? dme : eta;
+                eta = dmn > eta ? dmn : eta;
+                const double tj = face_tau_tab_t<true>(U0 * U0 + U1 * U1 + U2 * U2, eta, tau_lds);
+                const double sg = ((frec[i] >> 10) & 1) ? -1.0 : 1.0;
+                const double s0[3] = {sg * T0, sg * T1, sg * T2}, s1[3] = {sg * (tj * U0), sg * (tj * U1), sg * (tj * U2)};
+                const bool mine = i == 2 ? h == 1 : i == h;
+                const double (&Km)[9] = i == 2 ? KB : KA;
+                double (&Bm)[10][3] = i == 2 ? BB : BA;
+#pragma unroll
+                for (int t = 0; t < 3; ++t) {
+                    P[1 + 3 * i][t] = sg * (Ke[t * 3 + 0] * N0 + Ke[t * 3 + 1] * N1 + Ke[t * 3 + 2] * N2);
+                    P[2 + 3 * i][t] = s0[t];
+                    P[3 + 3 * i][t] = s1[t];
+                    const double nb = -sg * (Km[t * 3 + 0] * N0 + Km[t * 3 + 1] * N1 + Km[t * 3 + 2] * N2);
+                    Bm[1 + 3 * i][t] = mine ? nb : 0.0;
+                    Bm[2 + 3 * i][t] = mine ? -s0[t] : 0.0;
+                    Bm[3 + 3 * i][t] = mine ? -s1[t] : 0.0;
+                }
+            }
+            double g3[3], z[3];
+            front_panel(P, de, g3, z);
+            double *const stg = Nm + f * P6_STAGE_F;
+            apply_panel<3, false, true, true, false>(P, g3, BA);
+#pragma unroll
+            for (int t = 0; t < 3; ++t) uA[t] = fma(z[2], BA[2][t], fma(z[1], BA[1][t], z[0] * BA[0][t]));
+            if (p1) {
+#pragma unroll
+                for (int q = 0; q < 7; ++q) {
+#pragma unroll
+                    for (int t = 0; t < 3; ++t) stg[q * 10 + 3 * h + t] = BA[3 + q][t];
+                }
+            }
+            apply_panel<3, true, false, false, true>(P, g3, BB);
+#pragma unroll
+            for (int t = 0; t < 3; ++t) uB[t] = fma(z[2], BB[2][t], fma(z[1], BB[1][t], z[0] * BB[0][t]));
+            if (p1) {
+#pragma unroll
+                for (int q = 0; q < 7; ++q) stg[q * 10 + (h ? 6 : 9)] = BB[3 + q][0];
+                if (h) {
+#pragma unroll
+                    for (int q = 0; q < 7; ++q) { stg[q * 10 + 7] = BB[3 + q][1]; stg[q * 10 + 8] = BB[3 + q][2]; }
+                }
+            }
+        }
+        if (r < P6_D) { dbuf[3 * r + 0] = dod[0]; dbuf[3 * r + 1] = dod[1]; dbuf[3 * r + 2] = dod[2]; }
+        wave_lds_sync();
+
+        double C[P6_SLOTS][P6_NC + 1];
+#pragma unroll
+        for (int k = 0; k < P6_SLOTS; ++k) {
+            const int row = 16 * k + r;
+            const bool fill = row < 7 * P6_F;
+            const int ff = fill ? (row * 37) >> 8 : 0, d = row - 7 * P6_F;
+            const uint32_t q0 = dw[ff], q1 = dw[12 + ff];
+            const int s0 = (q0 >> 11) & 15, s1 = (q1 >> 6) & 15, s2 = (q1 >> 22) & 15;
+            const int fbase = ff * P6_STAGE_F + (row - 7 * ff) * 10;
+#pragma unroll
+            for (int sj = 0; sj < P6_D; ++sj) {
+                int off = P6_LDS_Z;
+                if (fill) {
+                    off = s0 == sj ? fbase : off;
+                    off = s1 == sj ? fbase + 3 : off;
+                    off = s2 == sj ? fbase + 6 : off;
+                } else {
+                    off = d == sj ? P6_LDS_D + 3 * sj : off;
+                }
+#pragma unroll
+                for (int t = 0; t < 3; ++t) C[k][3 * sj + t] = Nm[off + t];
+            }
+            C[k][P6_NC] = fill ? Nm[fbase + 9] : 1.0;
+        }
+        double rinv[2] = {0.0, 0.0};
+        p6_factor(C, rinv, r, std::make_integer_sequence<int, P6_NC>{});
+        const double c1 = r >= P6_NC - 16 ? C[1][P6_NC] : 0.0;
+        const double rr = row_allsum(fma(c1, c1, C[2][P6_NC] * C[2][P6_NC]));
+        {
+            double ct[2] = {C[0][P6_NC], C[1][P6_NC]}, y[2] = {0.0, 0.0};
+            p6_solve(C, rinv, ct, y, r, std::make_integer_sequence<int, P6_NC>{});
+            wave_lds_sync();
+            yb[r] = y[0];
+            if (r < P6_NC - 16) yb[16 + r] = y[1];
+        }
+        wave_lds_sync();
+        {
+            const int slA = (recA >> 6) & 15, slB = (frec[2] >> 6) & 15;
+            double part = fma(uA[2], yb[3 * slA + 2], fma(uA[1], yb[3 * slA + 1], uA[0] * yb[3 * slA]));
+            const double pb = fma(uB[2], yb[3 * slB + 2], fma(uB[1], yb[3 * slB + 1], uB[0] * yb[3 * slB]));
+            part += h ? pb : 1.0 - uB[0];
+            part += dpp_mov<0xB1>(part);
+            const double re = part;
+            const int ld = r < P6_D ? r : 0;
+            const double ro = 1.0 - fma(dod[2], yb[3 * ld + 2], fma(dod[1], yb[3 * ld + 1], dod[0] * yb[3 * ld]));
+            const double rri = fast_rcp(rr);
+            double we = re * rri, wo = ro * rri;
+            const bool ok = rr > 0.0;
+            we = (ok && __builtin_isfinite(we)) ? we : 0.0;
+            wo = (ok && __builtin_isfinite(wo)) ? wo : 0.0;
+            if (p1 && h == 0) wbuf[pe] = we;
+            if (r < P6_D) wbuf[po] = wo;
+        }
+        wave_lds_sync();
+        {
+            constexpr int ne = P6_F + P6_D;
+            const double nwv = is_neu ? wbuf[ne - 1] : 0.0;
+            const double addv = add_neumann ? nwv : 0.0;
+            if (valid && r < ne) out[eb + r] = wbuf[r] + addv;
+            if (valid && r == 0) nws[p] = nwv;
+        }
+        wave_lds_sync();
+    }
+}
+
+__global__ void k_prism6_flags(const uint32_t *__restrict__ desc, int32_t count, uint8_t *__restrict__ flags) {
+    const int64_t i = (int64_t)blockIdx.x * blockDim.x + threadIdx.x;
+    if (i >= count) return;
+    const uint32_t *dw = desc + (size_t)kMfwDescWords * i;
+    bool ok = (dw[24] & 0xFFFFFFu) == ((uint32_t)P6_F | ((uint32_t)P6_D << 8));
+    uint32_t deg = 0;
+    for (int f = 0; f < P6_F && ok; ++f) {
+        const uint32_t w0 = dw[f], w1 = dw[12 + f];
+        const uint32_t s[3] = {(w0 >> 11) & 15u, (w1 >> 6) & 15u, (w1 >> 22) & 15u};
+        for (int k = 0; k < 3; ++k) {
+            if (s[k] >= (uint32_t)P6_D) ok = false;
+            else deg += 1u << (4 * s[k]);
+        }
+    }
+    flags[i] = ok && deg == 0x333333u ? 1 : 0;
+}
+
+}
+
+int launch_prism6_flags(const uint32_t *desc, int32_t count, uint8_t *flags, hipStream_t stream) {
+    if (count <= 0) return 0;
+    hipLaunchKernelGGL(k_prism6_flags, dim3((unsigned)((count + 127) / 128)), dim3(128), 0, stream, desc, count, flags);
+    return hipGetLastError() == hipSuccess ? 0 : -3;
+}
+
+int launch_gls_prism6(const GridView &g, const int32_t *nodes, const uint32_t *desc, int32_t count, int add_neumann, double *out, double *nws,
+                      int32_t *queue, hipStream_t stream) {
+    if (count <= 0) return 0;
+    int64_t blocks = ((int64_t)count + 15) / 16;
+    const int64_t cap = 2 * 256;
+    if (blocks > cap) blocks = cap;
+    hipLaunchKernelGGL(nin_gls_prism6_kernel, dim3((unsigned)blocks), dim3(256), 0, stream, g, nodes, desc, count, add_neumann, out, nws, queue);
+    return hipGetLastError() == hipSuccess ? 0 : -3;
+}
+
+const char *kernel_name_gls_prism6() { return "nin_gls_prism6_kernel"; }
+
+}
diff --git a/ninpol_amd/csrc/launch.hpp b/ninpol_amd/csrc/launch.hpp
--- a/ninpol_amd/csrc/launch.hpp
+++ b/ninpol_amd/csrc/launch.hpp
@@ -43,6 +43,10 @@
 int launch_gls_mfw(const GridView &g, const int32_t *nodes, const uint32_t *desc, int32_t count, int kind, int add_neumann,
                    double *out, double *nws, int32_t *queue, hipStream_t stream);
 const char *kernel_name_gls_mfw();
+int launch_prism6_flags(const uint32_t *desc, int32_t count, uint8_t *flags, hipStream_t stream);
+int launch_gls_prism6(const GridView &g, const int32_t *nodes, const uint32_t *desc, int32_t count, int add_neumann, double *out, double *nws,
+                      int32_t *queue, hipStream_t stream);
+const char *kernel_name_gls_prism6();
 int launch_mfx_desc(const GridView &g, const int32_t *nodes, int32_t count, uint32_t *desc, hipStream_t stream);
 int launch_gls_mfx(const GridView &g, const int32_t *nodes, const uint32_t *desc, int32_t count, int cls, int add_neumann, double *out,
                    double *nws, int32_t *queue, hipStream_t stream);
diff --git a/ninpol_amd/grid.py b/ninpol_amd/grid.py
--- a/ninpol_amd/grid.py
+++ b/ninpol_amd/grid.py
@@ -348,6 +348,13 @@
         _lib.check(_lib.load().nin_gls_plan_flops(self._h, p(alg), p(ref), p(comp)))
         return {k: (float(alg[i]), float(ref[i]), int(comp[i])) for i, k in enumerate(self.PLAN_KERNELS)}
 
+    def gls_prism6_nodes(self):
+        n = ctypes.c_int64(0)
+        mask = np.zeros(int(self.n_points), dtype=np.uint8)
+        _lib.check(_lib.load().nin_gls_prism6_nodes(self._h, ctypes.byref(n), mask.ctypes.data_as(ctypes.c_void_p)))
+        assert int(mask.sum()) == n.value
+        return mask.astype(bool)
+
     def gls_plan(self):
         counts = np.zeros(22, dtype=np.int64)
         _lib.check(_lib.load().nin_gls_plan(self._h, counts.ctypes.data_as(ctypes.c_void_p)))
```

New measurement: 2287. Within noise of the previous version (-0.2%).
